# guptakhil/show-tell

Measured on AMD Instinct MI355X. Metric: training images/sec (ResNet101+GRU, emb=512, bs=128) at 1/2/4/8 MI355X, higher is better.
Workload: dtype bf16; 1 GPU; BASELINE configs[1]: ResNet-101 (train-mode BN, frozen) + 5-layer GRU decoder, E=H=512, V=10000, fwd+bwd+SGD step, synthetic COCO-shaped batch; batch_per_gpu=128, global_batch=128, image=3x224x224, parallelism=dp1

## Files before the change

include/showtell_hip.h:

```cpp
#ifndef SHOWTELL_HIP_H
#define SHOWTELL_HIP_H

#include <stddef.h>
#include <stdint.h>

#ifdef __cplusplus
extern "C" {
#endif

#define ST_F32 0
#define ST_BF16 1

#define ST_CELL_GRU 0
#define ST_CELL_LSTM 1

const char* st_last_error(void);
int st_version(void);

typedef struct {
  const void* x;
  const void* w;
  void* y;
  const float* bias;
  const float* scale;
  const float* shift;
  const void* residual;
  float* stats;
  int dtype, out_dtype;
  int B, Hin, Win, Cin, Ho, Wo, N, KH, KW, stride, pad;
  int ldx, ldw, ldy;
  int relu, accumulate;
  int Cin_logical;
  int k_order;
  int stats_replicas;
  const float* in_stats; const float* in_gamma; const float* in_beta; float in_count, in_eps;
  int split_k;
} st_conv_desc;

int st_conv(const st_conv_desc* d, void* stream);
int st_conv_batch(const st_conv_desc* d, int n, void* stream);

typedef struct {
  const void* x; const void* w_frag; void* y;
  float* stats; int stats_replicas;
  const float* scale; const float* shift; int relu;
  const float* in_stats; const float* in_gamma; const float* in_beta; float in_count; float in_eps;
  int B, H, W, C, N;
  int in_stats_replicas;
} st_conv3x3_img_desc;
int st_conv3x3_img_supported(int H, int W, int C, int N);
int st_conv3x3_img(const st_conv3x3_img_desc* d, void* stream);
int st_conv3x3_s2_supported(int C, int N);
int st_conv3x3_s2(const st_conv3x3_img_desc* d, void* stream);
typedef struct {
  const void* x; const void* w_frag; void* y; const void* residual;
  float* stats; int stats_replicas;
  const float* scale; const float* shift; int relu;
  const float* in_stats; const float* in_gamma; const float* in_beta; float in_count; float in_eps; int in_stats_replicas;
  int B, Hin, Win, C, N, stride;
} st_conv1x1_wreg_desc;
int st_conv1x1_wreg_supported(int C, int N);
int st_conv1x1_wreg(const st_conv1x1_wreg_desc* d, void* stream);
int st_conv1x1_kstream_supported(int C, int N);
int st_conv1x1_kstream(const st_conv1x1_wreg_desc* d, void* stream);
typedef struct {
  const void* raw; const void* identity; void* x_out; const void* w_frag; void* y;
  float* stats; int stats_replicas;
  const float* f_stats; const float* f_gamma; const float* f_beta; float f_count; float f_eps; int f_stats_replicas;
  long rows; int C, N;
  const float* id_stats; const float* id_gamma; const float* id_beta; int id_stats_replicas;
} st_conv1x1_kfuse_desc;
int st_conv1x1_kfuse_supported(int C, int N);
int st_conv1x1_kfuse(const st_conv1x1_kfuse_desc* d, void* stream);
#ifdef ST_EXPERIMENTAL
int st_conv1x1_kfuse8(const st_conv1x1_kfuse_desc* d, void* stream);
#endif
typedef struct {
  const void* raw2; const void* w3_frag; const void* identity; void* x_out; const void* w1_frag; void* y;
  float* stats; int stats_replicas;
  const float* bn2_stats; const float* bn2_gamma; const float* bn2_beta; int bn2_replicas;
  const float* bn3_stats; const float* bn3_gamma; const float* bn3_beta; int bn3_replicas;
  const float* id_stats; const float* id_gamma; const float* id_beta; int id_replicas;
  float count; float eps;
  long rows; int C1, C2, N;
} st_conv_b2b_desc;
int st_conv_b2b_supported(int C1, int C2, int N);
int st_conv_b2b(const st_conv_b2b_desc* d, void* stream);
typedef struct {
  const void* x2; const void* w3_frag; const void* identity; void* x_out; const void* w1_frag; void* y;
  float* stats; int stats_replicas;
  const float* bn2_stats; const float* bn2_gamma; const float* bn2_beta; int bn2_replicas;
  const float* bn3_stats; const float* bn3_gamma; const float* bn3_beta; int bn3_replicas;
  float count; float eps;
  const float* scale3; const float* shift3; const float* scale1; const float* shift1; int relu1;
  long rows; int C1, C2, N;
  const float* id_stats; const float* id_gamma; const float* id_beta; int id_replicas;
} st_conv_c3c1_desc;
int st_conv_c3c1_supported(int C1, int C2, int N);
int st_conv_c3c1(const st_conv_c3c1_desc* d, void* stream);
int st_conv1x1_astat_supported(int C, int N);
int st_conv1x1_astat(const st_conv1x1_wreg_desc* d, void* stream);

int st_pack_conv_weight_frag(const float* w, void* out, int Cout, int Cin, int KH, int KW, int ntw, void* stream);

int st_tune(int reserved, int kc, int w8);
int st_prof_enable(int on);
int st_debug_stamps(unsigned long long* buf);
int st_prof_collect(double* ms, double* flops, long* launches);

typedef struct {
  const void* x; void* y; const void* res;
  const float* stats;  const float* gamma; const float* beta;
  const float* running_mean; const float* running_var;
  const float* res_stats; const float* res_gamma; const float* res_beta;
  const float* res_running_mean; const float* res_running_var;
  int res_bn;
  int dtype; long rows; int C; float count; float eps; int relu;
  int stats_replicas, res_stats_replicas;
} st_bn_act_desc;

int st_bn_act(const st_bn_act_desc* d, void* stream);

int st_bn_update_running(const float* stats, float* running_mean, float* running_var,
                         int C, float count, float momentum, void* stream);

int st_nchw_to_nhwc(const float* x, void* y, int dtype, int B, int C, int H, int W, int Cpad, void* stream);
int st_nchw_to_s2d16(const float* x, void* y, int dtype, int B, int H, int W, void* stream);
int st_stem_weight_s2d(const void* w, void* out, int dtype, int Cpad, void* stream);
int st_nhwc_to_ncp_f32(const void* x, float* y, int dtype, int B, int HW, int C, void* stream);
int st_maxpool3x3s2(const void* x, void* y, int dtype, int B, int H, int W, int C, void* stream);
int st_maxpool3x3s2_bn(const void* x, void* y, int dtype, int B, int H, int W, int C,
                       const float* stats, const float* gamma, const float* beta,
                       const float* running_mean, const float* running_var, float count, float eps, void* stream);
typedef struct {
  const void* x_s2d; const void* w_frag; void* y;
  float* stats; int stats_replicas;
  const float* gamma;
  const float* scale; const float* shift;
  int B, H, W;
} st_stem_conv_pool_desc;
int st_stem_conv_pool(const st_stem_conv_pool_desc* d, void* stream);
int st_stem_weight_frag(const void* w_s2d, void* out, void* stream);
int st_stem_weight_frag_packed(const void* w_packed, int Cpad, void* out, void* stream);
int st_global_avgpool(const void* x, void* y, int dtype, int out_dtype, int B, int HW, int C, void* stream);

typedef struct st_image_batch_desc {
  const uint8_t* src;
  int64_t src_bytes;
  const int64_t* offset;
  const int32_t* height;
  const int32_t* width;
  const int32_t* flip;
  int batch;
  int max_height, max_width;
  int out_h, out_w;
  const float* lut;
  uint8_t* tmp;
  float* out;
  uint8_t* out_u8;
} st_image_batch_desc;
int st_image_transform(const st_image_batch_desc* d, void* stream);

int st_cast(const void* x, void* y, int from_dtype, int to_dtype, long n, void* stream);
int st_transpose(const void* x, void* y, int dtype, int rows, int cols, int ldx, int ldy, void* stream);
int st_transpose_colsum(const void* x, void* y, float* colsum, int dtype, int rows, int cols, int ldx, int ldy, void* stream);
int st_transpose_batch(const void* const* x, void* const* y, float* const* colsum, int n, int dtype, int rows, int cols,
                       int ldx, int ldy, const int* rows_t, const int* prev_row, void* stream);
int st_pack_conv_weight(const float* w, void* out, int dtype, int Cout, int Cin, int KH, int KW, int Cpad, int k_order, void* stream);

typedef struct st_resnet st_resnet;
int st_resnet_create(int version, int dtype, st_resnet** out);
void st_resnet_destroy(st_resnet* r);
int st_resnet_num_convs(const st_resnet* r);
int st_resnet_feat_dim(const st_resnet* r);
size_t st_resnet_weight_elems(const st_resnet* r);
size_t st_resnet_bn_channels(const st_resnet* r);
int st_resnet_conv_info(const st_resnet* r, int i, int* cin, int* cout, int* k, int* stride, int* pad,
                        int* cin_padded, size_t* weight_offset, size_t* bn_offset, int* k_order,
                        size_t* frag_weight_offset, int* frag_ntw);
size_t st_resnet_workspace_bytes(const st_resnet* r, int B, int H, int W);
int st_resnet_set_taps(st_resnet* r, void* buf, size_t bytes);
int st_resnet_forward(const st_resnet* r, const float* images_nchw, int B, int H, int W,
                      const void* weights, const float* bn_gamma, const float* bn_beta,
                      float* bn_running_mean, float* bn_running_var,
                      int train, float momentum, float eps,
                      void* workspace, size_t workspace_bytes,
                      void* feat_nhwc_out, void* pooled_out, int pooled_dtype, float* ncp_out,
                      void* stream);

int st_resnet_update_running(const st_resnet* r, const void* workspace, float* bn_running_mean, float* bn_running_var,
                             float momentum, void* stream);
int st_resnet_plan(const st_resnet* r, int B, int H, int W, int train, char* buf, size_t bytes);

int st_cast2d(const void* x, void* y, int from_dtype, int to_dtype, int rows, int cols, int ldx, int ldy, void* stream);

#define ST_MAX_LAYERS 8
typedef struct {
  int cell, dtype, L, in0, H, V, E;
  const void* emb;
  const void* w_ih[ST_MAX_LAYERS]; const void* w_hh[ST_MAX_LAYERS];
  const float* b_ih[ST_MAX_LAYERS]; const float* b_hh[ST_MAX_LAYERS];
  const void* w_lin; const float* b_lin;
} st_rnn_params;

typedef struct {
  float* emb;
  float* w_ih[ST_MAX_LAYERS]; float* w_hh[ST_MAX_LAYERS]; float* b_ih[ST_MAX_LAYERS]; float* b_hh[ST_MAX_LAYERS];
  float* w_lin; float* b_lin;
} st_rnn_grads;

typedef struct {
  int B, T, ntok, Tcap;
  const int* batch_sizes_host;
  const int* rows_b; const int* rows_t; const int* prev_row;
  const long* caption;
} st_packed_seq;

int st_rnn_vocab_ld(int V);
size_t st_rnn_workspace_bytes(const st_rnn_params* p, const st_packed_seq* s);
int st_rnn_forward(const st_rnn_params* p, const st_packed_seq* s, const void* x0_override, const void* feat,
                   void* workspace, size_t workspace_bytes, void* logits, int logits_dtype, int ldl,
                   long* targets, int save_for_backward, void* stream);
int st_rnn_backward(const st_rnn_params* p, const st_rnn_grads* g, const st_packed_seq* s,
                    const void* x0_override, const void* dlogits, int ldd, const float* dy_top,
                    void* workspace, size_t workspace_bytes, float* dfeat, float* dx0_out, void* stream);

int st_rnn_fused_loss_supported(const st_rnn_params* p);
size_t st_rnn_fused_loss_bytes(const st_rnn_params* p, const st_packed_seq* s);
int st_rnn_fused_loss(const st_rnn_params* p, const st_packed_seq* s, const void* workspace, size_t workspace_bytes,
                      const long* targets, float* scratch, size_t scratch_bytes, float* loss_accum, void* stream);
int st_rnn_fused_dlogits(const st_rnn_params* p, const st_packed_seq* s, const void* workspace, size_t workspace_bytes,
                         const long* targets, const float* scratch, const float* grad_scale_dev, void* dlogits, int ldd, void* stream);

int st_cross_entropy(const void* logits, int logits_dtype, const long* target, int rows, int V, int ldl,
                     float* loss_accum, void* dlogits, int dlogits_dtype, int ldd, float grad_scale,
                     const float* grad_scale_dev , void* stream);

size_t st_head_workspace_bytes(int B, int F, int E, int dtype);
int st_linear_bn1d_forward(const void* x, const void* w, const float* bias, const float* gamma, const float* beta,
                           float* running_mean, float* running_var, int B, int F, int E, int dtype,
                           int train, float momentum, float eps,
                           float* z_out, float* save_mean, float* save_rstd, void* y_dtype, float* y_f32, void* stream);
int st_linear_bn1d_backward(const float* dy, const float* z, const void* x, const float* gamma,
                            const float* save_mean, const float* save_rstd, int B, int F, int E, int dtype, int train,
                            float* dw, float* dbias, float* dgamma, float* dbeta, void* workspace, size_t workspace_bytes,
                            void* stream);

int st_sgd_step(float* param, const float* grad, float* momentum_buf, void* bf16_shadow, long n,
                float lr, float momentum, int first_step, float grad_scale, void* stream);
int st_adam_step(float* param, const float* grad, float* exp_avg, float* exp_avg_sq, void* bf16_shadow, long n,
                 float lr, float beta1, float beta2, float eps, int step, float grad_scale, void* stream);

size_t st_rnn_greedy_workspace_bytes(const st_rnn_params* p, int B);
int st_rnn_greedy(const st_rnn_params* p, const void* feat, int B, int steps, void* workspace, size_t workspace_bytes,
                  long* ids_out, float* logits_out, void* stream);
int st_rnn_greedy_last_route(void);

int st_rnn_step(const st_rnn_params* p, const void* x, int n, const void* h_in, const void* c_in,
                void* h_out, void* c_out, float* logits, int ldl, void* stream);
int st_embedding_rows(const void* emb, const long* ids, void* out, int n, int E, int V, int ldo, int dtype, void* stream);
int st_gather_state(const void* src, const int* idx, void* dst, int L, int n_src, int n_dst, int H, int dtype, void* stream);
int st_softmax_topk(const float* logits, int ldl, int n, int V, int k, float* top_p, long* top_id, int raw, void* stream);
int st_beam_select(const long* tok, const float* cost, uint8_t* done, const float* top_p, const long* top_id, int B, int W, int k,
                   long end_id, long* new_tok, float* new_cost, int* parent, uint8_t* ended, int* gather, void* stream);

int st_sample_rows(const float* logits, int ldl, int n, int V, const float* u, int u_stride, float inv_temperature, int top_k,
                   long end_id, uint8_t* finished, long* ids_out, float* logp_out, int out_stride, int t, long* cur, void* stream);
size_t st_rnn_sample_workspace_bytes(const st_rnn_params* p, int n);
int st_rnn_sample(const st_rnn_params* p, const void* feat, int n, int steps, const float* u, float inv_temperature, int top_k,
                  long end_id, void* workspace, size_t workspace_bytes, long* ids_out, float* logp_out, void* stream);

typedef struct {
  st_rnn_params rnn;
  int F, A, P;
  const void* w_enc; const float* b_enc;
  const void* w_dec; const float* b_dec;
  const float* w_full; const float* b_full;
  const void* w_init_h; const float* b_init_h;
  const void* w_init_c; const float* b_init_c;
  const void* w_embed; const float* b_embed;
} st_attn_params;

typedef struct {
  st_rnn_grads rnn;
  float *w_enc, *b_enc, *w_dec, *b_dec, *w_full, *b_full, *w_init_h, *b_init_h, *w_init_c, *b_init_c, *w_embed, *b_embed;
} st_attn_grads;

size_t st_attn_workspace_bytes(const st_attn_params* p, const st_packed_seq* s);
int st_attn_forward(const st_attn_params* p, const st_packed_seq* s, const float* cnn_feature, const long* caption_T,
                    void* workspace, size_t workspace_bytes, void* logits, int logits_dtype, int ldl,
                    float* alphas, int save_for_backward, void* stream);
int st_attn_backward(const st_attn_params* p, const st_attn_grads* g, const st_packed_seq* s, const long* caption_T,
                     const void* dlogits, int ldd, const float* alphas,
                     const float* dalphas ,
                     float alpha_c, const float* grad_scale_dev, void* workspace, size_t workspace_bytes, void* stream);
int st_attn_reg_loss(const float* alphas, int B, int T, int P, float alpha_c, float* loss_accum, void* stream);
size_t st_attn_greedy_workspace_bytes(const st_attn_params* p, int B);
int st_attn_greedy(const st_attn_params* p, const float* cnn_feature, int B, int steps, long start_id,
                   void* workspace, size_t workspace_bytes, long* ids_out, void* stream);
int st_attn_greedy_alphas(const st_attn_params* p, const float* cnn_feature, int B, int steps, long start_id,
                          void* workspace, size_t workspace_bytes, long* ids_out, float* alphas_out, void* stream);
size_t st_attn_sample_workspace_bytes(const st_attn_params* p, int n);
int st_attn_sample(const st_attn_params* p, const float* cnn_feature, int n, int steps, long start_id, const float* u,
                   float inv_temperature, int top_k, long end_id, void* workspace, size_t workspace_bytes,
                   long* ids_out, float* logp_out, float* alphas_out, void* stream);
size_t st_attn_beam_workspace_bytes(const st_attn_params* p, int B, int W);
int st_attn_beam_search(const st_attn_params* p, const float* cnn_feature, int B, int W, int max_length,
                        long start_id, long end_id, void* workspace, size_t workspace_bytes,
                        long* rec_tok, float* rec_cost, int* rec_par, uint8_t* rec_end, float* rec_alpha, void* stream);

#ifdef __cplusplus
}
#endif
#endif
```

show-tell_amd/_lib.py:

```python
import ctypes as C
import os

_HERE = os.path.dirname(os.path.abspath(__file__))
LIB_PATH = os.path.join(_HERE, "lib", "libshowtell_hip.so")

ST_F32, ST_BF16 = 0, 1
ST_CELL_GRU, ST_CELL_LSTM = 0, 1

c_p, c_i, c_f, c_l = C.c_void_p, C.c_int, C.c_float, C.c_long


class ConvDesc(C.Structure):
    _fields_ = [("x", c_p), ("w", c_p), ("y", c_p), ("bias", c_p), ("scale", c_p), ("shift", c_p),
                ("residual", c_p), ("stats", c_p), ("dtype", c_i), ("out_dtype", c_i),
                ("B", c_i), ("Hin", c_i), ("Win", c_i), ("Cin", c_i), ("Ho", c_i), ("Wo", c_i), ("N", c_i),
                ("KH", c_i), ("KW", c_i), ("stride", c_i), ("pad", c_i),
                ("ldx", c_i), ("ldw", c_i), ("ldy", c_i), ("relu", c_i), ("accumulate", c_i), ("Cin_logical", c_i), ("k_order", c_i), ("stats_replicas", c_i),
                ("in_stats", c_p), ("in_gamma", c_p), ("in_beta", c_p), ("in_count", c_f), ("in_eps", c_f), ("split_k", c_i)]


class Conv3x3ImgDesc(C.Structure):
    _fields_ = [("x", c_p), ("w_frag", c_p), ("y", c_p), ("stats", c_p), ("stats_replicas", c_i), ("scale", c_p), ("shift", c_p),
                ("relu", c_i), ("in_stats", c_p), ("in_gamma", c_p), ("in_beta", c_p), ("in_count", c_f), ("in_eps", c_f),
                ("B", c_i), ("H", c_i), ("W", c_i), ("C", c_i), ("N", c_i), ("in_stats_replicas", c_i)]


class Conv1x1WregDesc(C.Structure):
    _fields_ = [("x", c_p), ("w_frag", c_p), ("y", c_p), ("residual", c_p), ("stats", c_p), ("stats_replicas", c_i), ("scale", c_p),
                ("shift", c_p), ("relu", c_i), ("in_stats", c_p), ("in_gamma", c_p), ("in_beta", c_p), ("in_count", c_f), ("in_eps", c_f),
                ("in_stats_replicas", c_i), ("B", c_i), ("Hin", c_i), ("Win", c_i), ("C", c_i), ("N", c_i), ("stride", c_i)]


class Conv1x1KfuseDesc(C.Structure):
    _fields_ = [("raw", c_p), ("identity", c_p), ("x_out", c_p), ("w_frag", c_p), ("y", c_p), ("stats", c_p), ("stats_replicas", c_i),
                ("f_stats", c_p), ("f_gamma", c_p), ("f_beta", c_p), ("f_count", c_f), ("f_eps", c_f), ("f_stats_replicas", c_i),
                ("rows", c_l), ("C", c_i), ("N", c_i),
                ("id_stats", c_p), ("id_gamma", c_p), ("id_beta", c_p), ("id_stats_replicas", c_i)]


class StemConvPoolDesc(C.Structure):
    _fields_ = [("x_s2d", c_p), ("w_frag", c_p), ("y", c_p), ("stats", c_p), ("stats_replicas", c_i), ("gamma", c_p),
                ("scale", c_p), ("shift", c_p), ("B", c_i), ("H", c_i), ("W", c_i)]


class ConvB2bDesc(C.Structure):
    _fields_ = [("raw2", c_p), ("w3_frag", c_p), ("identity", c_p), ("x_out", c_p), ("w1_frag", c_p), ("y", c_p),
                ("stats", c_p), ("stats_replicas", c_i),
                ("bn2_stats", c_p), ("bn2_gamma", c_p), ("bn2_beta", c_p), ("bn2_replicas", c_i),
                ("bn3_stats", c_p), ("bn3_gamma", c_p), ("bn3_beta", c_p), ("bn3_replicas", c_i),
                ("id_stats", c_p), ("id_gamma", c_p), ("id_beta", c_p), ("id_replicas", c_i),
                ("count", c_f), ("eps", c_f), ("rows", c_l), ("C1", c_i), ("C2", c_i), ("N", c_i)]


class ConvC3c1Desc(C.Structure):
    _fields_ = [("x2", c_p), ("w3_frag", c_p), ("identity", c_p), ("x_out", c_p), ("w1_frag", c_p), ("y", c_p),
                ("stats", c_p), ("stats_replicas", c_i),
                ("bn2_stats", c_p), ("bn2_gamma", c_p), ("bn2_beta", c_p), ("bn2_replicas", c_i),
                ("bn3_stats", c_p), ("bn3_gamma", c_p), ("bn3_beta", c_p), ("bn3_replicas", c_i),
                ("count", c_f), ("eps", c_f),
                ("scale3", c_p), ("shift3", c_p), ("scale1", c_p), ("shift1", c_p), ("relu1", c_i),
                ("rows", c_l), ("C1", c_i), ("C2", c_i), ("N", c_i),
                ("id_stats", c_p), ("id_gamma", c_p), ("id_beta", c_p), ("id_replicas", c_i)]


class BnActDesc(C.Structure):
    _fields_ = [("x", c_p), ("y", c_p), ("res", c_p), ("stats", c_p), ("gamma", c_p), ("beta", c_p),
                ("running_mean", c_p), ("running_var", c_p), ("res_stats", c_p), ("res_gamma", c_p),
                ("res_beta", c_p), ("res_running_mean", c_p), ("res_running_var", c_p), ("res_bn", c_i),
                ("dtype", c_i), ("rows", c_l), ("C", c_i), ("count", c_f), ("eps", c_f), ("relu", c_i),
                ("stats_replicas", c_i), ("res_stats_replicas", c_i)]


ST_MAX_LAYERS = 8


class RnnParams(C.Structure):
    _fields_ = [("cell", c_i), ("dtype", c_i), ("L", c_i), ("in0", c_i), ("H", c_i), ("V", c_i), ("E", c_i),
                ("emb", c_p), ("w_ih", c_p * ST_MAX_LAYERS), ("w_hh", c_p * ST_MAX_LAYERS),
                ("b_ih", c_p * ST_MAX_LAYERS), ("b_hh", c_p * ST_MAX_LAYERS), ("w_lin", c_p), ("b_lin", c_p)]


class RnnGrads(C.Structure):
    _fields_ = [("emb", c_p), ("w_ih", c_p * ST_MAX_LAYERS), ("w_hh", c_p * ST_MAX_LAYERS),
                ("b_ih", c_p * ST_MAX_LAYERS), ("b_hh", c_p * ST_MAX_LAYERS), ("w_lin", c_p), ("b_lin", c_p)]


class AttnParams(C.Structure):
    _fields_ = [("rnn", RnnParams), ("F", c_i), ("A", c_i), ("P", c_i),
                ("w_enc", c_p), ("b_enc", c_p), ("w_dec", c_p), ("b_dec", c_p), ("w_full", c_p), ("b_full", c_p),
                ("w_init_h", c_p), ("b_init_h", c_p), ("w_init_c", c_p), ("b_init_c", c_p), ("w_embed", c_p), ("b_embed", c_p)]


class AttnGrads(C.Structure):
    _fields_ = [("rnn", RnnGrads)] + [(n, c_p) for n in ("w_enc", "b_enc", "w_dec", "b_dec", "w_full", "b_full", "w_init_h", "b_init_h",
                                                        "w_init_c", "b_init_c", "w_embed", "b_embed")]


class PackedSeq(C.Structure):
    _fields_ = [("B", c_i), ("T", c_i), ("ntok", c_i), ("Tcap", c_i), ("batch_sizes_host", C.POINTER(c_i)),
                ("rows_b", c_p), ("rows_t", c_p), ("prev_row", c_p), ("caption", c_p)]


class ImageBatchDesc(C.Structure):
    _fields_ = [("src", c_p), ("src_bytes", C.c_int64), ("offset", c_p), ("height", c_p), ("width", c_p), ("flip", c_p), ("batch", c_i),
                ("max_height", c_i), ("max_width", c_i), ("out_h", c_i), ("out_w", c_i), ("lut", c_p), ("tmp", c_p),
                ("out", c_p), ("out_u8", c_p)]


_SIGS = {
    "st_version": ([], c_i),
    "st_image_transform": ([C.POINTER(ImageBatchDesc), c_p], c_i),
    "st_conv": ([C.POINTER(ConvDesc), c_p], c_i),
    "st_conv_batch": ([C.POINTER(ConvDesc), c_i, c_p], c_i),
    "st_conv3x3_img_supported": ([c_i, c_i, c_i, c_i], c_i),
    "st_conv3x3_img": ([C.POINTER(Conv3x3ImgDesc), c_p], c_i),
    "st_conv3x3_s2_supported": ([c_i, c_i], c_i),
    "st_conv3x3_s2": ([C.POINTER(Conv3x3ImgDesc), c_p], c_i),
    "st_conv1x1_wreg_supported": ([c_i, c_i], c_i),
    "st_conv1x1_wreg": ([C.POINTER(Conv1x1WregDesc), c_p], c_i),
    "st_conv1x1_kfuse": ([C.POINTER(Conv1x1KfuseDesc), c_p], c_i),
    "st_conv1x1_kfuse_supported": ([c_i, c_i], c_i),
    "st_conv1x1_kfuse8": ([C.POINTER(Conv1x1KfuseDesc), c_p], c_i),
    "st_conv_b2b": ([C.POINTER(ConvB2bDesc), c_p], c_i),
    "st_conv_b2b_supported": ([c_i, c_i, c_i], c_i),
    "st_conv1x1_astat_supported": ([c_i, c_i], c_i),
    "st_conv1x1_astat": ([C.POINTER(Conv1x1WregDesc), c_p], c_i),
    "st_conv1x1_kstream_supported": ([c_i, c_i], c_i),
    "st_conv1x1_kstream": ([C.POINTER(Conv1x1WregDesc), c_p], c_i),
    "st_pack_conv_weight_frag": ([c_p, c_p, c_i, c_i, c_i, c_i, c_i, c_p], c_i),
    "st_tune": ([c_i, c_i, c_i], c_i),
    "st_prof_enable": ([c_i], c_i),
    "st_debug_stamps": ([c_p], c_i),
    "st_prof_collect": ([C.POINTER(C.c_double), C.POINTER(C.c_double), C.POINTER(c_l)], c_i),
    "st_bn_act": ([C.POINTER(BnActDesc), c_p], c_i),
    "st_bn_update_running": ([c_p, c_p, c_p, c_i, c_f, c_f, c_p], c_i),
    "st_nchw_to_nhwc": ([c_p, c_p, c_i, c_i, c_i, c_i, c_i, c_i, c_p], c_i),
    "st_nchw_to_s2d16": ([c_p, c_p, c_i, c_i, c_i, c_i, c_p], c_i),
    "st_stem_weight_s2d": ([c_p, c_p, c_i, c_i, c_p], c_i),
    "st_stem_weight_frag": ([c_p, c_p, c_p], c_i),
    "st_stem_weight_frag_packed": ([c_p, c_i, c_p, c_p], c_i),
    "st_stem_conv_pool": ([C.POINTER(StemConvPoolDesc), c_p], c_i),
    "st_nhwc_to_ncp_f32": ([c_p, c_p, c_i, c_i, c_i, c_i, c_p], c_i),
    "st_maxpool3x3s2": ([c_p, c_p, c_i, c_i, c_i, c_i, c_i, c_p], c_i),
    "st_maxpool3x3s2_bn": ([c_p, c_p, c_i, c_i, c_i, c_i, c_i, c_p, c_p, c_p, c_p, c_p, c_f, c_f, c_p], c_i),
    "st_global_avgpool": ([c_p, c_p, c_i, c_i, c_i, c_i, c_i, c_p], c_i),
    "st_cast": ([c_p, c_p, c_i, c_i, c_l, c_p], c_i),
    "st_transpose": ([c_p, c_p, c_i, c_i, c_i, c_i, c_i, c_p], c_i),
    "st_transpose_colsum": ([c_p, c_p, c_p, c_i, c_i, c_i, c_i, c_i, c_p], c_i),
    "st_transpose_batch": ([c_p, c_p, c_p, c_i, c_i, c_i, c_i, c_i, c_i, c_p, c_p, c_p], c_i),
    "st_pack_conv_weight": ([c_p, c_p, c_i, c_i, c_i, c_i, c_i, c_i, c_i, c_p], c_i),
    "st_cast2d": ([c_p, c_p, c_i, c_i, c_i, c_i, c_i, c_i, c_p], c_i),
    "st_rnn_vocab_ld": ([c_i], c_i),
    "st_rnn_workspace_bytes": ([C.POINTER(RnnParams), C.POINTER(PackedSeq)], C.c_size_t),
    "st_rnn_forward": ([C.POINTER(RnnParams), C.POINTER(PackedSeq), c_p, c_p, c_p, C.c_size_t, c_p, c_i, c_i, c_p, c_i, c_p], c_i),
    "st_rnn_fused_loss_supported": ([C.POINTER(RnnParams)], c_i),
    "st_rnn_fused_loss_bytes": ([C.POINTER(RnnParams), C.POINTER(PackedSeq)], C.c_size_t),
    "st_rnn_fused_loss": ([C.POINTER(RnnParams), C.POINTER(PackedSeq), c_p, C.c_size_t, c_p, c_p, C.c_size_t, c_p, c_p], c_i),
    "st_rnn_fused_dlogits": ([C.POINTER(RnnParams), C.POINTER(PackedSeq), c_p, C.c_size_t, c_p, c_p, c_p, c_p, c_i, c_p], c_i),
    "st_rnn_backward": ([C.POINTER(RnnParams), C.POINTER(RnnGrads), C.POINTER(PackedSeq), c_p, c_p, c_i, c_p, c_p, C.c_size_t,
                         c_p, c_p, c_p], c_i),
    "st_rnn_greedy_workspace_bytes": ([C.POINTER(RnnParams), c_i], C.c_size_t),
    "st_rnn_greedy": ([C.POINTER(RnnParams), c_p, c_i, c_i, c_p, C.c_size_t, c_p, c_p, c_p], c_i),
    "st_rnn_greedy_last_route": ([], c_i),
    "st_rnn_step": ([C.POINTER(RnnParams), c_p, c_i, c_p, c_p, c_p, c_p, c_p, c_i, c_p], c_i),
    "st_embedding_rows": ([c_p, c_p, c_p, c_i, c_i, c_i, c_i, c_i, c_p], c_i),
    "st_gather_state": ([c_p, c_p, c_p, c_i, c_i, c_i, c_i, c_i, c_p], c_i),
    "st_softmax_topk": ([c_p, c_i, c_i, c_i, c_i, c_p, c_p, c_i, c_p], c_i),
    "st_beam_select": ([c_p, c_p, c_p, c_p, c_p, c_i, c_i, c_i, c_l, c_p, c_p, c_p, c_p, c_p, c_p], c_i),
    "st_sample_rows": ([c_p, c_i, c_i, c_i, c_p, c_i, c_f, c_i, c_l, c_p, c_p, c_p, c_i, c_i, c_p, c_p], c_i),
    "st_rnn_sample_workspace_bytes": ([C.POINTER(RnnParams), c_i], C.c_size_t),
    "st_rnn_sample": ([C.POINTER(RnnParams), c_p, c_i, c_i, c_p, c_f, c_i, c_l, c_p, C.c_size_t, c_p, c_p, c_p], c_i),
    "st_attn_workspace_bytes": ([c_p, c_p], C.c_size_t),
    "st_attn_forward": ([c_p, c_p, c_p, c_p, c_p, C.c_size_t, c_p, c_i, c_i, c_p, c_i, c_p], c_i),
    "st_attn_backward": ([c_p, c_p, c_p, c_p, c_p, c_i, c_p, c_p, c_f, c_p, c_p, C.c_size_t, c_p], c_i),
    "st_attn_reg_loss": ([c_p, c_i, c_i, c_i, c_f, c_p, c_p], c_i),
    "st_attn_greedy_workspace_bytes": ([c_p, c_i], C.c_size_t),
    "st_attn_greedy": ([c_p, c_p, c_i, c_i, c_l, c_p, C.c_size_t, c_p, c_p], c_i),
    "st_attn_greedy_alphas": ([c_p, c_p, c_i, c_i, c_l, c_p, C.c_size_t, c_p, c_p, c_p], c_i),
    "st_attn_sample_workspace_bytes": ([c_p, c_i], C.c_size_t),
    "st_attn_sample": ([c_p, c_p, c_i, c_i, c_l, c_p, c_f, c_i, c_l, c_p, C.c_size_t, c_p, c_p, c_p, c_p], c_i),
    "st_attn_beam_workspace_bytes": ([c_p, c_i, c_i], C.c_size_t),
    "st_attn_beam_search": ([c_p, c_p, c_i, c_i, c_i, c_l, c_l, c_p, C.c_size_t, c_p, c_p, c_p, c_p, c_p, c_p], c_i),
    "st_cross_entropy": ([c_p, c_i, c_p, c_i, c_i, c_i, c_p, c_p, c_i, c_i, c_f, c_p, c_p], c_i),
    "st_head_workspace_bytes": ([c_i, c_i, c_i, c_i], C.c_size_t),
    "st_linear_bn1d_forward": ([c_p] * 7 + [c_i, c_i, c_i, c_i, c_i, c_f, c_f] + [c_p] * 6, c_i),
    "st_linear_bn1d_backward": ([c_p] * 6 + [c_i, c_i, c_i, c_i, c_i] + [c_p] * 5 + [C.c_size_t, c_p], c_i),
    "st_sgd_step": ([c_p, c_p, c_p, c_p, c_l, c_f, c_f, c_i, c_f, c_p], c_i),
    "st_adam_step": ([c_p, c_p, c_p, c_p, c_p, c_l, c_f, c_f, c_f, c_f, c_i, c_f, c_p], c_i),
    "st_resnet_create": ([c_i, c_i, C.POINTER(c_p)], c_i),
    "st_resnet_destroy": ([c_p], None),
    "st_resnet_num_convs": ([c_p], c_i),
    "st_resnet_feat_dim": ([c_p], c_i),
    "st_resnet_weight_elems": ([c_p], C.c_size_t),
    "st_resnet_bn_channels": ([c_p], C.c_size_t),
    "st_resnet_conv_info": ([c_p, c_i] + [C.POINTER(c_i)] * 6 + [C.POINTER(C.c_size_t)] * 2 + [C.POINTER(c_i), C.POINTER(C.c_size_t), C.POINTER(c_i)], c_i),
    "st_resnet_workspace_bytes": ([c_p, c_i, c_i, c_i], C.c_size_t),
    "st_resnet_set_taps": ([c_p, c_p, C.c_size_t], c_i),
    "st_resnet_forward": ([c_p, c_p, c_i, c_i, c_i, c_p, c_p, c_p, c_p, c_p, c_i, c_f, c_f, c_p, C.c_size_t,
                           c_p, c_p, c_i, c_p, c_p], c_i),
    "st_resnet_update_running": ([c_p, c_p, c_p, c_p, c_f, c_p], c_i),
    "st_resnet_plan": ([c_p, c_i, c_i, c_i, c_i, C.c_char_p, C.c_size_t], c_i),
}

_lib = None


class ShowTellHipError(RuntimeError):
    pass


def declared_symbols():
    return sorted([k for k in _SIGS if k not in _EXPERIMENTAL] + ["st_last_error"])


_EXPERIMENTAL = ("st_conv1x1_kfuse8",)


def has_symbol(name):
    return hasattr(lib(), name)


def lib():
    global _lib
    if _lib is None:
        if not os.path.isfile(LIB_PATH):
            raise ShowTellHipError(
                f"{LIB_PATH} not found: build it with `python -c 'import __graft_entry__ as g; g.build()'` "
                "(there is no CPU fallback for the HIP path)")
        import torch
        L = C.CDLL(LIB_PATH)
        L.st_last_error.restype = C.c_char_p
        L.st_last_error.argtypes = []
        for name, (args, res) in _SIGS.items():
            if name in _EXPERIMENTAL and not hasattr(L, name):
                continue
            fn = getattr(L, name)
            fn.argtypes, fn.restype = args, res
        _lib = L
    return _lib


def check(rc, what):
    if rc != 0:
        raise ShowTellHipError(f"{what}: {lib().st_last_error().decode()}")
```

show-tell_amd/csrc/rnn.cpp:

```cpp
#include "decoder_host.h"
#include <stdlib.h>

namespace {

struct Plan {
  int G, GH, Np, Vp, maxw;
  size_t es;
  size_t x0, y, gates, cst, dyl, dx0, dgx, dgh, dhc, dcc, tA, tB, wT, wThh, wTih, gA, gB, total;
};

Plan make_plan(const st_rnn_params* p, const st_packed_seq* s) {
  Plan q;
  q.G = p->cell == ST_CELL_GRU ? 3 : 4;
  q.GH = q.G * p->H;
  q.Np = st_up8(s->ntok);
  q.Vp = st_rnn_vocab_ld(p->V);
  q.es = st_dtype_size(p->dtype);
  q.maxw = p->in0 > p->H ? p->in0 : p->H;
  const size_t n = s->ntok, L = p->L, H = p->H;
  Arena ar;
  q.x0 = ar.take(n * p->in0 * q.es);
  q.y = ar.take(L * n * H * q.es);
  q.gates = ar.take(L * n * 4 * H * q.es);
  q.cst = ar.take(p->cell == ST_CELL_LSTM ? L * n * H * q.es : 0);
  q.dyl = ar.take(L * n * H * sizeof(float));
  q.dx0 = ar.take(n * p->in0 * sizeof(float));
  q.dgx = ar.take(L * n * q.GH * q.es);
  q.dgh = ar.take(p->cell == ST_CELL_GRU ? L * n * q.GH * q.es : 0);
  q.dhc = ar.take(L * (size_t)s->B * H * sizeof(float));
  q.dcc = ar.take(L * (size_t)s->B * H * sizeof(float));
  const size_t ra = (size_t)(p->V > q.GH ? p->V : q.GH);
  q.tA = ar.take(ra * q.Np * q.es);
  q.tB = ar.take((size_t)q.maxw * q.Np * q.es);
  const size_t w1 = (size_t)H * q.Vp, w2 = (size_t)q.maxw * q.GH;
  q.wT = ar.take((w1 > w2 ? w1 : w2) * q.es);
  q.wThh = ar.take(L * H * q.GH * q.es);
  q.wTih = ar.take(L * (size_t)q.maxw * q.GH * q.es);
  q.gA = ar.take(2 * L * (size_t)q.GH * q.Np * q.es);
  q.gB = ar.take(2 * L * (size_t)q.maxw * q.Np * q.es);
  q.total = ar.o;
  return q;
}

int check_common(const st_rnn_params* p, const st_packed_seq* s, const char* who) {
  ST_CHECK(p && s, "%s: null descriptor", who);
  ST_CHECK(p->cell == ST_CELL_GRU || p->cell == ST_CELL_LSTM, "%s: bad cell %d", who, p->cell);
  ST_CHECK(p->dtype == ST_F32 || p->dtype == ST_BF16, "%s: bad dtype %d", who, p->dtype);
  ST_CHECK(p->L >= 1 && p->L <= ST_MAX_LAYERS, "%s: num_layers=%d out of range [1,%d]", who, p->L, ST_MAX_LAYERS);
  ST_CHECK(p->H % 8 == 0 && p->in0 % 8 == 0 && p->E % 8 == 0, "%s: E=%d, in0=%d and H=%d must be multiples of 8", who, p->E, p->in0, p->H);
  ST_CHECK(p->V > 0, "%s: bad vocabulary size", who);
  if (st_check_packed_seq(s, who, true)) return 1;
  for (int l = 0; l < p->L; ++l)
    ST_CHECK(p->w_ih[l] && p->w_hh[l] && p->b_ih[l] && p->b_hh[l], "%s: null weights for layer %d", who, l);
  return 0;
}

}

extern "C" int st_rnn_vocab_ld(int V) { return V < 2048 ? st_up8(V) : (V + 511) / 512 * 512; }

extern "C" size_t st_rnn_workspace_bytes(const st_rnn_params* p, const st_packed_seq* s) {
  if (!p || !s) return 0;
  return make_plan(p, s).total;
}

extern "C" int st_rnn_forward(const st_rnn_params* p, const st_packed_seq* s, const void* x0_override, const void* feat,
                              void* workspace, size_t workspace_bytes, void* logits, int logits_dtype, int ldl,
                              long* targets, int save_for_backward, void* stream) {
  if (check_common(p, s, "st_rnn_forward")) return 1;
  ST_CHECK(workspace && (x0_override || (feat && p->emb)), "st_rnn_forward: null pointer");
  const Plan q = make_plan(p, s);
  ST_CHECK(workspace_bytes >= q.total, "st_rnn_forward: workspace too small (%zu < %zu)", workspace_bytes, q.total);
  hipStream_t st = reinterpret_cast<hipStream_t>(stream);
  char* ws = reinterpret_cast<char*>(workspace);
  const int dt = p->dtype, H = p->H, n = s->ntok;
  const size_t es = q.es;

  const void* x0 = x0_override;
  if (!x0) {
    ST_CHECK(p->in0 == p->E, "st_rnn_forward: in0 != E needs x0_override");
    if (pack_inputs_launch(feat, p->emb, s->caption, s->Tcap, s->rows_b, s->rows_t, ws + q.x0, targets, n, p->E, p->V, 0, dt, st)) return 1;
    x0 = ws + q.x0;
  }
  const std::vector<int> off = st_packed_offsets(s);

  const int L = p->L, T = s->T;
  for (int d = 0; d < T + L - 1; ++d) {
    RnnGemmArgs cells[ST_MAX_LAYERS];
    int nc = 0;
    for (int l = d < T ? 0 : d - (T - 1); l <= d && l < L; ++l) {
      const int t = d - l;
      const int bt = s->batch_sizes_host[t];
      const char* xl = l == 0 ? reinterpret_cast<const char*>(x0) : ws + q.y + (size_t)(l - 1) * n * H * es;
      const int in = l == 0 ? p->in0 : H;
      char* yl = ws + q.y + (size_t)l * n * H * es;
      char* gl = ws + q.gates + (size_t)l * n * 4 * H * es;
      char* cl = ws + q.cst + (size_t)l * n * H * es;
      cells[nc++] = rnn_full_cell(p, l, xl + (size_t)off[t] * in * es, in, t > 0 ? yl + (size_t)off[t - 1] * H * es : nullptr,
                                  t > 0 ? cl + (size_t)off[t - 1] * H * es : nullptr, yl + (size_t)off[t] * H * es, cl + (size_t)off[t] * H * es,
                                  bt, save_for_backward ? gl + (size_t)off[t] * 4 * H * es : nullptr);
    }
    if (rnn_gemm_launch_batch(cells, nc, dt, rnn_cell_epi(p->cell), 1, st)) return 1;
  }
  if (logits) {
    ST_CHECK(p->w_lin && p->b_lin, "st_rnn_forward: logits requested without the vocabulary projection");
    const char* ytop = ws + q.y + (size_t)(p->L - 1) * n * H * es;
    if (st_gemm_nt(ytop, H, p->w_lin, H, logits, ldl, n, p->V, H, dt, logits_dtype, p->b_lin, stream)) return 1;
  }
  return 0;
}

extern "C" int st_rnn_fused_loss_supported(const st_rnn_params* p) {
  return p && p->w_lin && p->b_lin && vocab_ce_supported(p->dtype, p->H) ? 1 : 0;
}
extern "C" size_t st_rnn_fused_loss_bytes(const st_rnn_params* p, const st_packed_seq* s) {
  if (!p || !s) return 0;
  return ((size_t)s->ntok * (2 + 2 * (size_t)vocab_ce_tiles(p->V))) * sizeof(float);
}
extern "C" int st_rnn_fused_loss(const st_rnn_params* p, const st_packed_seq* s, const void* workspace, size_t workspace_bytes,
                                 const long* targets, float* scratch, size_t scratch_bytes, float* loss_accum, void* stream) {
  if (check_common(p, s, "st_rnn_fused_loss")) return 1;
  ST_CHECK(workspace && targets && scratch && loss_accum, "st_rnn_fused_loss: null pointer");
  ST_CHECK(st_rnn_fused_loss_supported(p), "st_rnn_fused_loss: needs bf16, H = 512 and the vocabulary projection (use st_rnn_forward's logits + st_cross_entropy)");
  const Plan q = make_plan(p, s);
  ST_CHECK(workspace_bytes >= q.total && scratch_bytes >= st_rnn_fused_loss_bytes(p, s), "st_rnn_fused_loss: workspace / scratch too small");
  const char* ytop = reinterpret_cast<const char*>(workspace) + q.y + (size_t)(p->L - 1) * s->ntok * p->H * q.es;
  const int n = s->ntok;
  return vocab_ce_forward(ytop, p->w_lin, p->b_lin, targets, n, p->V, scratch + 2 * (size_t)n, scratch + n, scratch, loss_accum,
                          reinterpret_cast<hipStream_t>(stream));
}
extern "C" int st_rnn_fused_dlogits(const st_rnn_params* p, const st_packed_seq* s, const void* workspace, size_t workspace_bytes,
                                    const long* targets, const float* scratch, const float* grad_scale_dev, void* dlogits, int ldd, void* stream) {
  if (check_common(p, s, "st_rnn_fused_dlogits")) return 1;
  ST_CHECK(workspace && targets && scratch && dlogits, "st_rnn_fused_dlogits: null pointer");
  ST_CHECK(st_rnn_fused_loss_supported(p), "st_rnn_fused_dlogits: unsupported configuration");
  const Plan q = make_plan(p, s);
  ST_CHECK(workspace_bytes >= q.total, "st_rnn_fused_dlogits: workspace too small");
  const char* ytop = reinterpret_cast<const char*>(workspace) + q.y + (size_t)(p->L - 1) * s->ntok * p->H * q.es;
  return vocab_ce_dlogits(ytop, p->w_lin, p->b_lin, targets, scratch, s->ntok, p->V, dlogits, ldd, 1.0f, grad_scale_dev,
                          reinterpret_cast<hipStream_t>(stream));
}

extern "C" int st_rnn_backward(const st_rnn_params* p, const st_rnn_grads* g, const st_packed_seq* s,
                               const void* x0_override, const void* dlogits, int ldd, const float* dy_top_extra,
                               void* workspace, size_t workspace_bytes, float* dfeat, float* dx0_out, void* stream) {
  if (check_common(p, s, "st_rnn_backward")) return 1;
  ST_CHECK(g && workspace, "st_rnn_backward: null pointer");
  const Plan q = make_plan(p, s);
  ST_CHECK(workspace_bytes >= q.total, "st_rnn_backward: workspace too small (%zu < %zu)", workspace_bytes, q.total);
  hipStream_t st = reinterpret_cast<hipStream_t>(stream);
  char* ws = reinterpret_cast<char*>(workspace);
  const int dt = p->dtype, H = p->H, n = s->ntok, Np = q.Np, GH = q.GH;
  const size_t es = q.es;
  const std::vector<int> off = st_packed_offsets(s);
  const int L = p->L, T = s->T;
  auto dyl = [&](int l) { return reinterpret_cast<float*>(ws + q.dyl) + (size_t)l * n * H; };
  float* dy = dyl(L - 1);
  const char* ytop = ws + q.y + (size_t)(p->L - 1) * n * H * es;

  if (dlogits) {
    ST_CHECK(p->w_lin && g->w_lin && g->b_lin, "st_rnn_backward: vocabulary projection gradients requested without buffers");
    ST_CHECK(ldd >= st_up8(p->V) && ldd % 8 == 0 && ldd <= q.Vp, "st_rnn_backward: dlogits leading dimension %d must be a multiple of 8 in [%d, %d]",
             ldd, st_up8(p->V), q.Vp);
    if (st_transpose_colsum(dlogits, ws + q.tA, g->b_lin, dt, n, p->V, ldd, Np, stream)) return 1;
    if (st_transpose(ytop, ws + q.tB, dt, n, H, H, Np, stream)) return 1;
    if (st_gemm_nt(ws + q.tA, Np, ws + q.tB, Np, g->w_lin, H, p->V, H, Np, dt, ST_F32, nullptr, stream, 1)) return 1;
    if (st_transpose(p->w_lin, ws + q.wT, dt, p->V, H, H, ldd, stream)) return 1;
    const int bk = dt == ST_BF16 ? 64 : 32;
    const int split = (ldd % (8 * bk) == 0 && ldd >= 16 * bk) ? 8 : 0;
    if (st_gemm_nt(dlogits, ldd, ws + q.wT, ldd, dy, H, n, H, ldd, dt, ST_F32, nullptr, stream, 0, split)) return 1;
    if (dy_top_extra) { st_set_error("st_rnn_backward: dlogits and dy_top_extra are exclusive"); return 1; }
  } else {
    ST_CHECK(dy_top_extra, "st_rnn_backward: need dlogits or dy_top");
    if (hipMemcpyAsync(dy, dy_top_extra, (size_t)n * H * sizeof(float), hipMemcpyDeviceToDevice, st) != hipSuccess) {
      st_set_error("st_rnn_backward: copy failed"); return 1;
    }
  }

  const void* x0 = x0_override ? x0_override : ws + q.x0;
  const bool need_dx0 = dfeat || dx0_out || g->emb;
  float* dx0 = dx0_out ? dx0_out : reinterpret_cast<float*>(ws + q.dx0);
  const bool gru = p->cell == ST_CELL_GRU;
  auto dgxl = [&](int l) { return ws + q.dgx + (size_t)l * n * GH * es; };
  auto dghl = [&](int l) { return gru ? ws + q.dgh + (size_t)l * n * GH * es : dgxl(l); };
  auto dhcl = [&](int l) { return reinterpret_cast<float*>(ws + q.dhc) + (size_t)l * s->B * H; };
  auto dccl = [&](int l) { return reinterpret_cast<float*>(ws + q.dcc) + (size_t)l * s->B * H; };
  auto wThh = [&](int l) { return ws + q.wThh + (size_t)l * H * GH * es; };
  auto wTih = [&](int l) { return ws + q.wTih + (size_t)l * q.maxw * GH * es; };
  if (hipMemsetAsync(ws + q.dhc, 0, (size_t)L * s->B * H * sizeof(float), st) != hipSuccess ||
      hipMemsetAsync(ws + q.dcc, 0, (size_t)L * s->B * H * sizeof(float), st) != hipSuccess) { st_set_error("memset failed"); return 1; }
  {
    const void* wx[2][ST_MAX_LAYERS]; void* wy[2][ST_MAX_LAYERS];
    int ni = 0;
    for (int l = 0; l < L; ++l) {
      const int in = l == 0 ? p->in0 : H;
      wx[0][l] = p->w_hh[l]; wy[0][l] = wThh(l);
      if (!(l > 0 || need_dx0)) continue;
      if (in == H) { wx[1][ni] = p->w_ih[l]; wy[1][ni] = wTih(l); ++ni; }
      else if (st_transpose(p->w_ih[l], wTih(l), dt, GH, in, in, GH, stream)) return 1;
    }
    if (st_transpose_batch(wx[0], wy[0], nullptr, L, dt, GH, H, H, GH, nullptr, nullptr, stream)) return 1;
    if (ni && st_transpose_batch(wx[1], wy[1], nullptr, ni, dt, GH, H, H, GH, nullptr, nullptr, stream)) return 1;
  }
  auto bwd_cell = [&](int l, int t, const float* dyrows) {
    const char* yl = ws + q.y + (size_t)l * n * H * es;
    const char* gl = ws + q.gates + (size_t)l * n * 4 * H * es;
    const char* cl = ws + q.cst + (size_t)l * n * H * es;
    RnnBwdCell c;
    memset(&c, 0, sizeof(c));
    c.dy = dyrows ? dyrows + (size_t)off[t] * H : nullptr; c.dhc = dhcl(l); c.dcc = dccl(l);
    c.cache = gl + (size_t)off[t] * 4 * H * es;
    c.hprev = t > 0 ? yl + (size_t)off[t - 1] * H * es : nullptr;
    c.cnew = cl + (size_t)off[t] * H * es;
    c.cprev = t > 0 ? cl + (size_t)off[t - 1] * H * es : nullptr;
    c.dgx = dgxl(l) + (size_t)off[t] * GH * es; c.dgh = dghl(l) + (size_t)off[t] * GH * es; c.Bt = s->batch_sizes_host[t];
    return c;
  };
  const char* env = getenv("ST_BPTT_FUSED");
  const bool fused = !(env && env[0] == '0');
  for (int d = T + L - 2; fused && d >= 0; --d) {
    RnnBwdFused fc[ST_MAX_LAYERS];
    int nf = 0;
    for (int l = d < T ? 0 : d - (T - 1); l <= d && l < L; ++l) {
      const int t = d - l;
      RnnBwdFused& f = fc[nf++];
      memset(&f, 0, sizeof(f));
      f.e = bwd_cell(l, t, l == L - 1 ? dy : nullptr);
      RnnGemmArgs& a = f.g;
      a.M = f.e.Bt; a.N = H;
      if (t + 1 < T) {
        a.A = dghl(l) + (size_t)off[t + 1] * GH * es; a.W = wThh(l); a.M2 = s->batch_sizes_host[t + 1]; a.K = GH; a.lda = GH; a.ldw = GH;
      }
      if (l + 1 < L) {
        a.A2 = dgxl(l + 1) + (size_t)off[t] * GH * es; a.W2 = wTih(l + 1); a.K2 = GH; a.lda2 = GH; a.ldw2 = GH;
      }
    }
    if (rnn_bwd_fused_launch_batch(fc, nf, p->cell, dt, st)) return 1;
  }
  if (fused && need_dx0 && st_gemm_nt(dgxl(0), GH, wTih(0), GH, dx0, p->in0, n, p->in0, GH, dt, ST_F32, nullptr, stream)) return 1;
  for (int d = T + L - 2; !fused && d >= 0; --d) {
    RnnBwdCell gc[ST_MAX_LAYERS];
    RnnGemmArgs mc[2 * ST_MAX_LAYERS];
    int ng = 0, nm = 0;
    for (int l = d < T ? 0 : d - (T - 1); l <= d && l < L; ++l) {
      const int t = d - l;
      const int bt = s->batch_sizes_host[t];
      const int in = l == 0 ? p->in0 : H;
      gc[ng++] = bwd_cell(l, t, dyl(l));
      if (t > 0) {
        RnnGemmArgs& a = mc[nm++];
        memset(&a, 0, sizeof(a));
        a.A = dghl(l) + (size_t)off[t] * GH * es; a.W = wThh(l); a.M = bt; a.N = H; a.K = GH; a.lda = GH; a.ldw = GH;
        a.out_f32 = dhcl(l); a.ldo = H; a.accumulate = 1;
      }
      if (l > 0 || need_dx0) {
        RnnGemmArgs& a = mc[nm++];
        memset(&a, 0, sizeof(a));
        a.A = dgxl(l) + (size_t)off[t] * GH * es; a.W = wTih(l); a.M = bt; a.N = in; a.K = GH; a.lda = GH; a.ldw = GH;
        a.out_f32 = (l > 0 ? dyl(l - 1) + (size_t)off[t] * H : dx0 + (size_t)off[t] * in); a.ldo = in;
      }
    }
    if (rnn_bwd_gates_launch_batch(gc, ng, H, p->cell, dt, st)) return 1;
    if (rnn_gemm_launch_batch(mc, nm, dt, 0, 0, st)) return 1;
  }
  st_conv_desc gd[2 * ST_MAX_LAYERS];
  int ng = 0;
  auto wgrad = [&](const void* aT, const void* bT, float* dw, int rows, int cols) {
    gd[ng++] = st_gemm_nt_desc(aT, Np, bT, Np, dw, cols, rows, cols, Np, dt, ST_F32, nullptr, 1);
  };
  const void* tx[4][ST_MAX_LAYERS]; void* ty[4][ST_MAX_LAYERS]; float* tc[4][ST_MAX_LAYERS];
  int nx = 0;
  for (int l = 0; l < L; ++l) {
    const int in = l == 0 ? p->in0 : H;
    const char* xl = l == 0 ? reinterpret_cast<const char*>(x0) : ws + q.y + (size_t)(l - 1) * n * H * es;
    char* aIh = ws + q.gA + (size_t)(2 * l) * GH * Np * es;
    char* aHh = ws + q.gA + (size_t)(2 * l + 1) * GH * Np * es;
    char* bIh = ws + q.gB + (size_t)(2 * l) * q.maxw * Np * es;
    char* bHh = ws + q.gB + (size_t)(2 * l + 1) * q.maxw * Np * es;
    tx[0][l] = dgxl(l); ty[0][l] = aIh; tc[0][l] = g->b_ih[l];
    tx[2][l] = dghl(l); ty[2][l] = aHh; tc[2][l] = g->b_hh[l];
    tx[3][l] = ws + q.y + (size_t)l * n * H * es; ty[3][l] = bHh; tc[3][l] = nullptr;
    if (in == H) {
      tx[1][nx] = xl; ty[1][nx] = bIh; tc[1][nx] = nullptr; ++nx;
      wgrad(aIh, bIh, g->w_ih[l], GH, in);
    } else {
      if (st_transpose(xl, bIh, dt, n, in, in, Np, stream)) return 1;
    }
    wgrad(gru ? aHh : aIh, bHh, g->w_hh[l], GH, H);
    if (!gru && colsum_launch(dghl(l), g->b_hh[l], n, GH, GH, dt, st)) return 1;
  }
  if (st_transpose_batch(tx[0], ty[0], tc[0], L, dt, n, GH, GH, Np, nullptr, nullptr, stream)) return 1;
  if (nx && st_transpose_batch(tx[1], ty[1], nullptr, nx, dt, n, H, H, Np, nullptr, nullptr, stream)) return 1;
  if (gru && st_transpose_batch(tx[2], ty[2], tc[2], L, dt, n, GH, GH, Np, nullptr, nullptr, stream)) return 1;
  if (st_transpose_batch(tx[3], ty[3], nullptr, L, dt, n, H, H, Np, s->rows_t, s->prev_row, stream)) return 1;
  for (int l = 0; l < L; ++l) {
    const int in = l == 0 ? p->in0 : H;
    if (in != H && st_gemm_nt(ws + q.gA + (size_t)(2 * l) * GH * Np * es, Np, ws + q.gB + (size_t)(2 * l) * q.maxw * Np * es, Np,
                              g->w_ih[l], in, GH, in, Np, dt, ST_F32, nullptr, stream, 1)) return 1;
  }
  for (int i = 0; i < ng; i += 12) {
    if (st_conv_batch(gd + i, ng - i < 12 ? ng - i : 12, stream)) return 1;
  }
  if (need_dx0 && !x0_override) {
    ST_CHECK(g->emb, "st_rnn_backward: embedding gradient buffer missing");
    if (embedding_bwd_launch(dx0, s->caption, s->Tcap, s->rows_b, s->rows_t, dfeat, g->emb, n, p->E, p->V, 0, st)) return 1;
  }
  return 0;
}
```

show-tell_amd/csrc/rnn_kernels.h:

```cpp
#pragma once
#include "common.h"

struct RnnGemmArgs {
  const void* A; const void* W; int M, N, K, lda, ldw, gstride;
  const void* A2; const void* W2; int K2, lda2, ldw2;
  int M2;
  float* out_f32; int ldo; int accumulate;
  const float* bias_h; const float* bias_x;
  const void* gx; int ldgx;
  const void* hprev; const void* cprev; int ldhp;
  void* hout; void* cout; int ldho;
  void* hout2; int ldho2;
  void* cache; int ldcache;
  unsigned long long* argmax_keys;
  const unsigned long long* x_keys; int x_V;
  long* ids_out; int ids_stride, ids_t;
};
constexpr int kCellRawOut = 1, kCellSplit = 2;

constexpr int kRnnBatch = 16;
struct RnnGemmBatch { RnnGemmArgs c[kRnnBatch]; };
static_assert(sizeof(RnnGemmBatch) <= 4000, "kernel-argument segment is 4 KiB");
struct RnnBwdCell {
  const float* dy; float* dhc; float* dcc; const void* cache; const void* hprev; const void* cnew; const void* cprev;
  void* dgx; void* dgh; int Bt;
};
struct RnnBwdBatch { RnnBwdCell c[kRnnBatch]; };
struct RnnBwdFused { RnnGemmArgs g; RnnBwdCell e; };
struct RnnBwdFusedBatch { RnnBwdFused c[ST_MAX_LAYERS]; };
static_assert(sizeof(RnnBwdFusedBatch) <= 4000, "kernel-argument segment is 4 KiB");

#ifdef __HIPCC__
__device__ __forceinline__ float st_sigm(float x) { return 1.0f / (1.0f + expf(-x)); }
__device__ __forceinline__ float st_gru_unit(float xr, float xz, float xn, float hr, float hz, float hn, float hprev, float& r, float& z, float& n) {
  r = st_sigm(xr + hr);
  z = st_sigm(xz + hz);
  n = tanhf(__builtin_fmaf(r, hn, xn));
  return __builtin_fmaf(z, hprev, (1.f - z) * n);
}
__device__ __forceinline__ float st_lstm_unit(float pi, float pf, float pg, float po, float cprev, float& ig, float& fg, float& gg, float& og, float& cn) {
  ig = st_sigm(pi); fg = st_sigm(pf); gg = tanhf(pg); og = st_sigm(po);
  cn = __builtin_fmaf(fg, cprev, ig * gg);
  return og * tanhf(cn);
}
#endif

size_t rnn_greedy_pipe_bytes(const st_rnn_params* p, int B, int steps);
int rnn_greedy_pipe(const st_rnn_params* p, const void* feat, int B, int steps, void* ws, size_t ws_bytes, long* ids_out, hipStream_t st);

int vocab_ce_supported(int dtype, int H);
int vocab_ce_tiles(int V);
int vocab_ce_forward(const void* y, const void* w, const float* bias, const long* target, int n, int V, float* partial, float* tgt,
                     float* lse, float* loss, hipStream_t st);
int vocab_ce_dlogits(const void* y, const void* w, const float* bias, const long* target, const float* lse, int n, int V,
                     void* dlogits, int ldd, float gscale, const float* gscale_dev, hipStream_t st);

int rnn_gemm_launch(const RnnGemmArgs& a, int dtype, int epi, int has_x, hipStream_t st);
int rnn_gemm_launch_batch(const RnnGemmArgs* cells, int ncells, int dtype, int epi, int has_x, hipStream_t st);
int rnn_bwd_gates_launch_batch(const RnnBwdCell* cells, int ncells, int H, int cell_kind, int dtype, hipStream_t st);
int rnn_bwd_fused_launch_batch(const RnnBwdFused* cells, int ncells, int cell_kind, int dtype, hipStream_t st);
int pack_inputs_launch(const void* feat, const void* emb, const long* cap, int Tcap, const int* rows_b, const int* rows_t,
                       void* x0, long* target, int ntok, int E, int V, int mode, int dtype, hipStream_t st);
int embedding_bwd_launch(const float* dx0, const long* cap, int Tcap, const int* rows_b, const int* rows_t,
                         float* dfeat, float* demb, int ntok, int E, int V, int mode, hipStream_t st);
int gather_hprev_launch(const void* y, const int* rows_t, const int* prev_row, void* hp, int ntok, int H, int dtype, hipStream_t st,
                        const void* h0 = nullptr, const int* rows_b = nullptr);
int gru_bwd_gates_launch(const float* dy, float* dhc, const void* cache, const void* hprev, void* dgx, void* dgh,
                         int Bt, int H, int dtype, hipStream_t st);
int lstm_bwd_gates_launch(const float* dy, float* dhc, float* dcc, const void* cache, const void* cnew, const void* cprev,
                          void* dg, int Bt, int H, int dtype, hipStream_t st);
int colsum_launch(const void* x, float* out, int rows, int cols, int ldx, int dtype, hipStream_t st);
```

show-tell_amd/csrc/rnn_kernels.hip:

```cpp
#include "common.h"
#include "rnn_kernels.h"
#include <string.h>

namespace {

template <typename T> struct Mfma;
template <> struct Mfma<bf16_t> {
  static constexpr int EPC = 8;
  static __device__ __forceinline__ void run(const u32x4& a, const u32x4& b, f32x4& c) {
    c = __builtin_amdgcn_mfma_f32_16x16x32_bf16(*reinterpret_cast<const bf16x8*>(&a),
                                                *reinterpret_cast<const bf16x8*>(&b), c, 0, 0, 0);
  }
};
template <> struct Mfma<float> {
  static constexpr int EPC = 4;
  static __device__ __forceinline__ void run(const u32x4& a, const u32x4& b, f32x4& c) {
#pragma unroll
    for (int e = 0; e < 4; ++e)
      c = __builtin_amdgcn_mfma_f32_16x16x4f32(__uint_as_float(a[e]), __uint_as_float(b[e]), c, 0, 0, 0);
  }
};

template <typename T> __device__ __forceinline__ void load4(const T* p, float* v);
template <> __device__ __forceinline__ void load4<float>(const float* p, float* v) {
  const f32x4 t = *reinterpret_cast<const f32x4*>(p);
  v[0] = t[0]; v[1] = t[1]; v[2] = t[2]; v[3] = t[3];
}
template <> __device__ __forceinline__ void load4<bf16_t>(const bf16_t* p, float* v) {
  const u32x2 t = *reinterpret_cast<const u32x2*>(p);
  v[0] = __uint_as_float(t[0] << 16); v[1] = __uint_as_float(t[0] & 0xffff0000u);
  v[2] = __uint_as_float(t[1] << 16); v[3] = __uint_as_float(t[1] & 0xffff0000u);
}
template <typename T> __device__ __forceinline__ void store4(T* p, const float* v);
template <> __device__ __forceinline__ void store4<float>(float* p, const float* v) {
  *reinterpret_cast<f32x4*>(p) = f32x4{v[0], v[1], v[2], v[3]};
}
template <> __device__ __forceinline__ void store4<bf16_t>(bf16_t* p, const float* v) {
  *reinterpret_cast<u32x2*>(p) = u32x2{pack_bf16x2(v[0], v[1]), pack_bf16x2(v[2], v[3])};
}

__device__ __forceinline__ float sigm(float x) { return 1.0f / (1.0f + expf(-x)); }

__device__ __forceinline__ u32x4 lane_gather(const u32x4& v, int src4) {
  return u32x4{(unsigned)__builtin_amdgcn_ds_bpermute(src4, (int)v[0]), (unsigned)__builtin_amdgcn_ds_bpermute(src4, (int)v[1]),
               (unsigned)__builtin_amdgcn_ds_bpermute(src4, (int)v[2]), (unsigned)__builtin_amdgcn_ds_bpermute(src4, (int)v[3])};
}
template <typename T, int NG, bool HAS_X, int MT, bool BWD = false>
__device__ __forceinline__ void skinny_mma(const RnnGemmArgs& a, int mbase, int n0, int r16, int q4, int kslice,
                                           f32x4 (&accH)[MT][NG], f32x4 (&accX)[MT][NG]) {
  constexpr int EPC = Mfma<T>::EPC;
  constexpr int UNR = BWD ? (MT + NG <= 4 ? 4 : 2) : (HAS_X && MT == 2) ? 2 : 4;
  const int lr = BWD ? q4 * 4 + (r16 >> 2) : r16, lq = BWD ? (r16 & 3) : q4;
  const int n = n0 + lr;
  const bool nok = n < a.N;
  const bool hasH = a.A != nullptr, hasX = HAS_X && a.A2 != nullptr;
  const T* WH = reinterpret_cast<const T*>(a.W) + (long)n * a.ldw;
  const long gsH = (long)a.gstride * a.ldw;
  const T* WX = reinterpret_cast<const T*>(a.W2) + (long)n * a.ldw2;
  const long gsX = (long)a.gstride * a.ldw2;
  const T* AH[MT]; const T* AX[MT]; bool mok[MT], mokH[MT];
#pragma unroll
  for (int t = 0; t < MT; ++t) {
    const int m = mbase + t * 16 + lr;
    mok[t] = m < a.M;
    mokH[t] = BWD ? m < a.M2 : mok[t];
    AH[t] = reinterpret_cast<const T*>(a.A) + (long)m * a.lda;
    if (!HAS_X && a.x_keys && a.A) {
      int tok = 0;
      if (mok[t]) {
        tok = (int)(0xffffffffu - (unsigned)(a.x_keys[m] & 0xffffffffull));
        if (tok < 0 || tok >= a.x_V) tok = 0;
        if (a.ids_out && n0 == 0 && kslice == 0 && q4 == 0) a.ids_out[(long)m * a.ids_stride + a.ids_t] = tok;
      }
      AH[t] = reinterpret_cast<const T*>(a.A) + (long)tok * a.lda;
    }
    long xrow = m;
    if (HAS_X && a.x_keys) {
      int tok = 0;
      if (mok[t]) {
        tok = (int)(0xffffffffu - (unsigned)(a.x_keys[m] & 0xffffffffull));
        if (tok < 0 || tok >= a.x_V) tok = 0;
        if (a.ids_out && n0 == 0 && kslice == 0 && q4 == 0) a.ids_out[(long)m * a.ids_stride + a.ids_t] = tok;
      }
      xrow = tok;
    }
    AX[t] = reinterpret_cast<const T*>(a.A2) + xrow * a.lda2;
  }
  const int nsH = hasH ? (a.K + 4 * EPC - 1) / (4 * EPC) : 0, nsX = hasX ? (a.K2 + 4 * EPC - 1) / (4 * EPC) : 0;
  const int spwH = (nsH + 3) / 4, spwX = (nsX + 3) / 4;
  const int begH = kslice * spwH, endH = min(nsH, begH + spwH), begX = kslice * spwX, endX = min(nsX, begX + spwX);
  const int ngroups = max((endH - begH + UNR - 1) / UNR, (endX - begX + UNR - 1) / UNR);
  for (int gi = 0; gi < ngroups; ++gi) {
    u32x4 fa[MT][UNR], fw[UNR][NG], xa[MT][UNR], xw[UNR][NG];
#pragma unroll
    for (int u = 0; u < UNR; ++u) {
      const int sH = begH + gi * UNR + u, kH = (sH * 4 + lq) * EPC;
      const bool okH = sH < endH && kH < a.K;
#pragma unroll
      for (int t = 0; t < MT; ++t) {
        fa[t][u] = u32x4{0u, 0u, 0u, 0u};
        if (mokH[t] && okH) fa[t][u] = *reinterpret_cast<const u32x4*>(AH[t] + kH);
      }
#pragma unroll
      for (int g = 0; g < NG; ++g) {
        fw[u][g] = u32x4{0u, 0u, 0u, 0u};
        if ((BWD ? n + g * 16 < a.N : nok) && okH) fw[u][g] = *reinterpret_cast<const u32x4*>(WH + g * gsH + kH);
      }
      if (HAS_X) {
        const int sX = begX + gi * UNR + u, kX = (sX * 4 + lq) * EPC;
        const bool okX = sX < endX && kX < a.K2;
#pragma unroll
        for (int t = 0; t < MT; ++t) {
          xa[t][u] = u32x4{0u, 0u, 0u, 0u};
          if (mok[t] && okX) xa[t][u] = *reinterpret_cast<const u32x4*>(AX[t] + kX);
        }
#pragma unroll
        for (int g = 0; g < NG; ++g) {
          xw[u][g] = u32x4{0u, 0u, 0u, 0u};
          if ((BWD ? n + g * 16 < a.N : nok) && okX) xw[u][g] = *reinterpret_cast<const u32x4*>(WX + g * gsX + kX);
        }
      }
    }
    if (BWD) {
      const int src4 = (r16 * 4 + q4) * 4;
#pragma unroll
      for (int u = 0; u < UNR; ++u) {
#pragma unroll
        for (int t = 0; t < MT; ++t) { fa[t][u] = lane_gather(fa[t][u], src4); xa[t][u] = lane_gather(xa[t][u], src4); }
#pragma unroll
        for (int g = 0; g < NG; ++g) { fw[u][g] = lane_gather(fw[u][g], src4); xw[u][g] = lane_gather(xw[u][g], src4); }
      }
    }
#pragma unroll
    for (int u = 0; u < UNR; ++u)
#pragma unroll
      for (int g = 0; g < NG; ++g)
#pragma unroll
        for (int t = 0; t < MT; ++t) {
          Mfma<T>::run(fw[u][g], fa[t][u], accH[t][g]);
          if (HAS_X) Mfma<T>::run(xw[u][g], xa[t][u], accX[t][g]);
        }
  }
}

template <typename T, int NG, int EPI, bool HAS_X, int MT>
__global__ __launch_bounds__(256) void rnn_gemm_kernel(RnnGemmBatch batch) {
  const RnnGemmArgs& a = batch.c[blockIdx.z];
  __shared__ f32x4 red[4][MT][2 * NG][64];
  const int lane = threadIdx.x & 63;
  const int wid = __builtin_amdgcn_readfirstlane(threadIdx.x >> 6);
  const int r16 = lane & 15, q4 = lane >> 4;
  const int n0 = blockIdx.x * 16, mbase = blockIdx.y * 16 * MT;
  if (mbase >= a.M || n0 >= a.N) return;
  const int m0 = mbase + (wid < MT ? wid : 0) * 16;
  f32x4 accH[MT][NG], accX[MT][NG];
#pragma unroll
  for (int t = 0; t < MT; ++t)
#pragma unroll
    for (int g = 0; g < NG; ++g) { accH[t][g] = f32x4{0.f, 0.f, 0.f, 0.f}; accX[t][g] = f32x4{0.f, 0.f, 0.f, 0.f}; }
  const int pm = m0 + r16, pn = n0 + 4 * q4;
  const bool epi_ok = wid < MT && pm < a.M && pn < a.N && EPI != 3;
  float ex[NG][4], eb[NG][4], es[4] = {0.f, 0.f, 0.f, 0.f};
#pragma unroll
  for (int g = 0; g < NG; ++g)
#pragma unroll
    for (int e = 0; e < 4; ++e) { ex[g][e] = 0.f; eb[g][e] = 0.f; }
  if (epi_ok) {
    if (EPI == 0) {
      if (a.bias_h) load4<float>(a.bias_h + pn, eb[0]);
      if (a.accumulate) load4<float>(a.out_f32 + (long)pm * a.ldo + pn, es);
    } else {
#pragma unroll
      for (int g = 0; g < NG; ++g) {
        load4<float>(a.bias_h + g * a.N + pn, eb[g]);
        if (HAS_X) load4<float>(a.bias_x + g * a.N + pn, ex[g]);
        else if (a.accumulate == kCellSplit) load4<float>(reinterpret_cast<const float*>(a.gx) + (long)pm * a.ldgx + g * a.N + pn, ex[g]);
        else if (a.accumulate != kCellRawOut) load4<T>(reinterpret_cast<const T*>(a.gx) + (long)pm * a.ldgx + g * a.N + pn, ex[g]);
      }
      const void* prev = EPI == 1 ? a.hprev : a.cprev;
      if (prev && a.accumulate != kCellRawOut) load4<T>(reinterpret_cast<const T*>(prev) + (long)pm * a.ldhp + pn, es);
    }
  }
  skinny_mma<T, NG, HAS_X, MT>(a, mbase, n0, r16, q4, wid, accH, accX);
#pragma unroll
  for (int t = 0; t < MT; ++t)
#pragma unroll
    for (int g = 0; g < NG; ++g) { red[wid][t][g][lane] = accH[t][g]; if (HAS_X) red[wid][t][NG + g][lane] = accX[t][g]; }
  __syncthreads();
  if (wid >= MT) return;
  f32x4 sumH[NG], sumX[NG];
#pragma unroll
  for (int g = 0; g < NG; ++g) {
    sumH[g] = red[0][wid][g][lane];
    if (HAS_X) sumX[g] = red[0][wid][NG + g][lane];
#pragma unroll
    for (int w = 1; w < 4; ++w) {
      sumH[g] += red[w][wid][g][lane];
      if (HAS_X) sumX[g] += red[w][wid][NG + g][lane];
    }
  }

  const int m = m0 + r16, n = n0 + 4 * q4;
  if (EPI != 3 && (m >= a.M || n >= a.N)) return;
  const int H = a.N;
  if (EPI == 3) {
    float best = -INFINITY; int bi = 0x7fffffff;
#pragma unroll
    for (int e = 0; e < 4; ++e) {
      if (n + e < a.N) {
        const float v = sumH[0][e] + (a.bias_h ? a.bias_h[n + e] : 0.f);
        if (v > best) { best = v; bi = n + e; }
      }
    }
#pragma unroll
    for (int o = 16; o < 64; o <<= 1) {
      const float ov = __shfl_xor(best, o, 64); const int oi = __shfl_xor(bi, o, 64);
      if (ov > best || (ov == best && oi < bi)) { best = ov; bi = oi; }
    }
    if (q4 == 0 && bi != 0x7fffffff && m < a.M) {
      unsigned u = __float_as_uint(best);
      u = (u & 0x80000000u) ? ~u : (u | 0x80000000u);
      const unsigned long long key = ((unsigned long long)u << 32) | (unsigned long long)(0xffffffffu - (unsigned)bi);
      atomicMax(a.argmax_keys + m, key);
    }
    return;
  }
  if (EPI == 0) {
    float v[4];
#pragma unroll
    for (int e = 0; e < 4; ++e) v[e] = sumH[0][e] + eb[0][e] + es[e];
    if (a.hout) store4<T>(reinterpret_cast<T*>(a.hout) + (long)m * a.ldho + n, v);
    else *reinterpret_cast<f32x4*>(a.out_f32 + (long)m * a.ldo + n) = f32x4{v[0], v[1], v[2], v[3]};
  } else if (!HAS_X && a.accumulate == kCellRawOut) {
#pragma unroll
    for (int g = 0; g < NG; ++g)
      *reinterpret_cast<f32x4*>(a.out_f32 + (long)m * a.ldo + g * a.N + n) =
          f32x4{sumH[g][0] + eb[g][0], sumH[g][1] + eb[g][1], sumH[g][2] + eb[g][2], sumH[g][3] + eb[g][3]};
  } else if (EPI == 1) {
    float xg[3][4];
    const float* hp = es;
    const bool split = !HAS_X && a.accumulate == kCellSplit;
#pragma unroll
    for (int g = 0; g < 3; ++g)
#pragma unroll
      for (int e = 0; e < 4; ++e) xg[g][e] = split ? sumH[g][e] + eb[g][e] : (HAS_X ? sumX[g][e] : 0.f) + ex[g][e];
    float hn[4], r[4], z[4], nn[4], hnew[4];
#pragma unroll
    for (int e = 0; e < 4; ++e) {
      const float hr = split ? ex[0][e] : sumH[0][e] + eb[0][e], hz = split ? ex[1][e] : sumH[1][e] + eb[1][e];
      hn[e] = split ? ex[2][e] : sumH[2][e] + eb[2][e];
      hnew[e] = st_gru_unit(xg[0][e], xg[1][e], xg[2][e], hr, hz, hn[e], hp[e], r[e], z[e], nn[e]);
    }
    store4<T>(reinterpret_cast<T*>(a.hout) + (long)m * a.ldho + n, hnew);
    if (a.hout2) store4<T>(reinterpret_cast<T*>(a.hout2) + (long)m * a.ldho2 + n, hnew);
    if (a.cache) {
      T* c = reinterpret_cast<T*>(a.cache) + (long)m * a.ldcache + n;
      store4<T>(c, r); store4<T>(c + H, z); store4<T>(c + 2 * H, nn); store4<T>(c + 3 * H, hn);
    }
  } else {
    float pre[4][4];
    const float* cp = es;
#pragma unroll
    for (int g = 0; g < 4; ++g)
#pragma unroll
      for (int e = 0; e < 4; ++e) pre[g][e] = (HAS_X ? sumX[g][e] : 0.f) + ex[g < NG ? g : 0][e] + sumH[g < NG ? g : 0][e] + eb[g < NG ? g : 0][e];
    float ig[4], fg[4], gg[4], og[4], cn[4], hnew[4];
#pragma unroll
    for (int e = 0; e < 4; ++e) hnew[e] = st_lstm_unit(pre[0][e], pre[1][e], pre[2][e], pre[3][e], cp[e], ig[e], fg[e], gg[e], og[e], cn[e]);
    store4<T>(reinterpret_cast<T*>(a.hout) + (long)m * a.ldho + n, hnew);
    if (a.hout2) store4<T>(reinterpret_cast<T*>(a.hout2) + (long)m * a.ldho2 + n, hnew);
    store4<T>(reinterpret_cast<T*>(a.cout) + (long)m * a.ldho + n, cn);
    if (a.cache) {
      T* c = reinterpret_cast<T*>(a.cache) + (long)m * a.ldcache + n;
      store4<T>(c, ig); store4<T>(c + H, fg); store4<T>(c + 2 * H, gg); store4<T>(c + 3 * H, og);
    }
  }
}

template <typename T>
__global__ __launch_bounds__(256) void pack_inputs_kernel(const T* __restrict__ feat, const T* __restrict__ emb,
                                                          const long* __restrict__ cap, int Tcap,
                                                          const int* __restrict__ rows_b, const int* __restrict__ rows_t,
                                                          T* __restrict__ x0, long* __restrict__ target,
                                                          int ntok, int E, int V, int mode) {
  constexpr int N = 16 / (int)sizeof(T);
  const int cpr = E / N;
  const long total = (long)ntok * cpr;
  for (long i = (long)blockIdx.x * blockDim.x + threadIdx.x; i < total; i += (long)gridDim.x * blockDim.x) {
    const int row = (int)(i / cpr), c = (int)(i - (long)row * cpr) * N;
    const int b = rows_b[row], t = rows_t[row];
    const T* src;
    if (mode == 0 && t == 0) src = feat + (long)b * E + c;
    else {
      long tok = cap[(long)b * Tcap + (mode == 0 ? t - 1 : t)];
      tok = tok < 0 ? 0 : (tok >= V ? V - 1 : tok);
      src = emb + tok * E + c;
    }
    *reinterpret_cast<u32x4*>(x0 + (long)row * E + c) = *reinterpret_cast<const u32x4*>(src);
    if (c == 0 && target) target[row] = cap[(long)b * Tcap + t];
  }
}

__global__ __launch_bounds__(256) void embedding_bwd_kernel(const float* __restrict__ dx0, const long* __restrict__ cap, int Tcap,
                                                            const int* __restrict__ rows_b, const int* __restrict__ rows_t,
                                                            float* __restrict__ dfeat, float* __restrict__ demb,
                                                            int ntok, int E, int V, int mode) {
  const long total = (long)ntok * E;
  for (long i = (long)blockIdx.x * blockDim.x + threadIdx.x; i < total; i += (long)gridDim.x * blockDim.x) {
    const int row = (int)(i / E), c = (int)(i - (long)row * E);
    const int b = rows_b[row], t = rows_t[row];
    const float v = dx0[i];
    if (mode == 0 && t == 0) { if (dfeat) dfeat[(long)b * E + c] = v; }
    else {
      long tok = cap[(long)b * Tcap + (mode == 0 ? t - 1 : t)];
      tok = tok < 0 ? 0 : (tok >= V ? V - 1 : tok);
      atomicAdd(demb + tok * E + c, v);
    }
  }
}

template <typename T>
__global__ __launch_bounds__(256) void gather_hprev_kernel(const T* __restrict__ y, const int* __restrict__ rows_t,
                                                           const int* __restrict__ prev_row, T* __restrict__ hp, int ntok, int H,
                                                           const T* __restrict__ h0, const int* __restrict__ rows_b) {
  constexpr int N = 16 / (int)sizeof(T);
  const int cpr = H / N;
  const long total = (long)ntok * cpr;
  for (long i = (long)blockIdx.x * blockDim.x + threadIdx.x; i < total; i += (long)gridDim.x * blockDim.x) {
    const int row = (int)(i / cpr), c = (int)(i - (long)row * cpr) * N;
    u32x4 v = {0u, 0u, 0u, 0u};
    if (rows_t[row] > 0) v = *reinterpret_cast<const u32x4*>(y + (long)prev_row[row] * H + c);
    else if (h0) v = *reinterpret_cast<const u32x4*>(h0 + (long)rows_b[row] * H + c);
    *reinterpret_cast<u32x4*>(hp + (long)row * H + c) = v;
  }
}

template <typename T>
__global__ __launch_bounds__(256) void gru_bwd_gates_kernel(RnnBwdBatch batch, int H) {
  const RnnBwdCell& cl = batch.c[blockIdx.y];
  const float* __restrict__ dy = cl.dy; float* __restrict__ dhc = cl.dhc;
  const T* __restrict__ cache = reinterpret_cast<const T*>(cl.cache);
  const T* __restrict__ hprev = reinterpret_cast<const T*>(cl.hprev);
  T* __restrict__ dgx = reinterpret_cast<T*>(cl.dgx); T* __restrict__ dgh = reinterpret_cast<T*>(cl.dgh);
  const int Bt = cl.Bt;
  const int total = Bt * (H / 4);
  const int i = blockIdx.x * blockDim.x + threadIdx.x;
  if (i >= total) return;
  const int b = i / (H / 4), j = (i - b * (H / 4)) * 4;
  float g[4], c[4], r[4], z[4], n[4], hn[4], hp[4] = {0.f, 0.f, 0.f, 0.f};
  load4<float>(dy + (long)b * H + j, g);
  load4<float>(dhc + (long)b * H + j, c);
  const T* cr = cache + (long)b * 4 * H + j;
  load4<T>(cr, r); load4<T>(cr + H, z); load4<T>(cr + 2 * H, n); load4<T>(cr + 3 * H, hn);
  if (hprev) load4<T>(hprev + (long)b * H + j, hp);
  float drp[4], dzp[4], dnp[4], dnr[4], dhz[4];
#pragma unroll
  for (int e = 0; e < 4; ++e) {
    const float dh = g[e] + c[e];
    const float dn = dh * (1.f - z[e]);
    const float dz = dh * (hp[e] - n[e]);
    dnp[e] = dn * (1.f - n[e] * n[e]);
    drp[e] = dnp[e] * hn[e] * r[e] * (1.f - r[e]);
    dzp[e] = dz * z[e] * (1.f - z[e]);
    dnr[e] = dnp[e] * r[e];
    dhz[e] = dh * z[e];
  }
  T* ox = dgx + (long)b * 3 * H + j;
  T* oh = dgh + (long)b * 3 * H + j;
  store4<T>(ox, drp); store4<T>(ox + H, dzp); store4<T>(ox + 2 * H, dnp);
  store4<T>(oh, drp); store4<T>(oh + H, dzp); store4<T>(oh + 2 * H, dnr);
  store4<float>(dhc + (long)b * H + j, dhz);
}

template <typename T>
__global__ __launch_bounds__(256) void lstm_bwd_gates_kernel(RnnBwdBatch batch, int H) {
  const RnnBwdCell& cl = batch.c[blockIdx.y];
  const float* __restrict__ dy = cl.dy; float* __restrict__ dhc = cl.dhc; float* __restrict__ dcc = cl.dcc;
  const T* __restrict__ cache = reinterpret_cast<const T*>(cl.cache);
  const T* __restrict__ cnew = reinterpret_cast<const T*>(cl.cnew);
  const T* __restrict__ cprev = reinterpret_cast<const T*>(cl.cprev);
  T* __restrict__ dg = reinterpret_cast<T*>(cl.dgx);
  const int Bt = cl.Bt;
  const int total = Bt * (H / 4);
  const int i = blockIdx.x * blockDim.x + threadIdx.x;
  if (i >= total) return;
  const int b = i / (H / 4), j = (i - b * (H / 4)) * 4;
  float g[4], ch[4], cc[4], ig[4], fg[4], gg[4], og[4], cn[4], cp[4] = {0.f, 0.f, 0.f, 0.f};
  load4<float>(dy + (long)b * H + j, g);
  load4<float>(dhc + (long)b * H + j, ch);
  load4<float>(dcc + (long)b * H + j, cc);
  const T* cr = cache + (long)b * 4 * H + j;
  load4<T>(cr, ig); load4<T>(cr + H, fg); load4<T>(cr + 2 * H, gg); load4<T>(cr + 3 * H, og);
  load4<T>(cnew + (long)b * H + j, cn);
  if (cprev) load4<T>(cprev + (long)b * H + j, cp);
  float di[4], df[4], dgg[4], dob[4], dcp[4], zero[4] = {0.f, 0.f, 0.f, 0.f};
#pragma unroll
  for (int e = 0; e < 4; ++e) {
    const float dh = g[e] + ch[e];
    const float tc = tanhf(cn[e]);
    const float dc = cc[e] + dh * og[e] * (1.f - tc * tc);
    dob[e] = dh * tc * og[e] * (1.f - og[e]);
    di[e] = dc * gg[e] * ig[e] * (1.f - ig[e]);
    df[e] = dc * cp[e] * fg[e] * (1.f - fg[e]);
    dgg[e] = dc * ig[e] * (1.f - gg[e] * gg[e]);
    dcp[e] = dc * fg[e];
  }
  T* o = dg + (long)b * 4 * H + j;
  store4<T>(o, di); store4<T>(o + H, df); store4<T>(o + 2 * H, dgg); store4<T>(o + 3 * H, dob);
  store4<float>(dcc + (long)b * H + j, dcp);
  store4<float>(dhc + (long)b * H + j, zero);
}


template <typename T> struct Raw4;
template <> struct Raw4<float> { typedef f32x4 type; };
template <> struct Raw4<bf16_t> { typedef u32x2 type; };
template <typename T> __device__ __forceinline__ void unpack4(const typename Raw4<T>::type& t, float* v);
template <> __device__ __forceinline__ void unpack4<float>(const f32x4& t, float* v) { v[0] = t[0]; v[1] = t[1]; v[2] = t[2]; v[3] = t[3]; }
template <> __device__ __forceinline__ void unpack4<bf16_t>(const u32x2& t, float* v) {
  v[0] = __uint_as_float(t[0] << 16); v[1] = __uint_as_float(t[0] & 0xffff0000u);
  v[2] = __uint_as_float(t[1] << 16); v[3] = __uint_as_float(t[1] & 0xffff0000u);
}

template <typename T, bool LSTM, int MT, int NT>
__global__ __launch_bounds__(256) void rnn_bwd_cell_kernel(RnnBwdFusedBatch batch) {
  typedef typename Raw4<T>::type raw_t;
  const RnnGemmArgs& a = batch.c[blockIdx.z].g;
  const RnnBwdCell& c = batch.c[blockIdx.z].e;
  constexpr int TILES = MT * NT, TPW = (TILES + 3) / 4;
  __shared__ f32x4 red[4][TILES][64];
  const int lane = threadIdx.x & 63;
  const int wid = __builtin_amdgcn_readfirstlane(threadIdx.x >> 6);
  const int r16 = lane & 15, q4 = lane >> 4;
  const int n0 = blockIdx.x * 16 * NT, mbase = blockIdx.y * 16 * MT;
  if (mbase >= a.M || n0 >= a.N) return;
  const int H = a.N;
  f32x4 accH[MT][NT], accX[MT][NT];
#pragma unroll
  for (int t = 0; t < MT; ++t)
#pragma unroll
    for (int g = 0; g < NT; ++g) { accH[t][g] = f32x4{0.f, 0.f, 0.f, 0.f}; accX[t][g] = f32x4{0.f, 0.f, 0.f, 0.f}; }
  bool ok[TPW]; int pm[TPW], pn[TPW];
  f32x4 rdy[TPW], rdhc[TPW], rdcc[TPW]; raw_t rc[TPW][4], rp[TPW], rcn[TPW];
  const T* cache = reinterpret_cast<const T*>(c.cache);
#pragma unroll
  for (int j = 0; j < TPW; ++j) {
    const int i = wid + 4 * j;
    pm[j] = mbase + (i / NT) * 16 + r16; pn[j] = n0 + (i % NT) * 16 + 4 * q4;
    ok[j] = i < TILES && pm[j] < a.M && pn[j] < H;
    rdy[j] = rdhc[j] = rdcc[j] = f32x4{0.f, 0.f, 0.f, 0.f};
    rp[j] = rcn[j] = raw_t{};
#pragma unroll
    for (int q = 0; q < 4; ++q) rc[j][q] = raw_t{};
    if (!ok[j]) continue;
    const long o = (long)pm[j] * H + pn[j];
    if (c.dy) rdy[j] = *reinterpret_cast<const f32x4*>(c.dy + o);
#pragma unroll
    for (int q = 0; q < 4; ++q) rc[j][q] = *reinterpret_cast<const raw_t*>(cache + (long)pm[j] * 4 * H + q * H + pn[j]);
    if (LSTM) {
      rdcc[j] = *reinterpret_cast<const f32x4*>(c.dcc + o);
      rcn[j] = *reinterpret_cast<const raw_t*>(reinterpret_cast<const T*>(c.cnew) + o);
      if (c.cprev) rp[j] = *reinterpret_cast<const raw_t*>(reinterpret_cast<const T*>(c.cprev) + o);
    } else {
      rdhc[j] = *reinterpret_cast<const f32x4*>(c.dhc + o);
      if (c.hprev) rp[j] = *reinterpret_cast<const raw_t*>(reinterpret_cast<const T*>(c.hprev) + o);
    }
  }
  skinny_mma<T, NT, true, MT, true>(a, mbase, n0, r16, q4, wid, accH, accX);
#pragma unroll
  for (int t = 0; t < MT; ++t)
#pragma unroll
    for (int g = 0; g < NT; ++g) red[wid][t * NT + g][lane] = accH[t][g] + accX[t][g];
  __syncthreads();
#pragma unroll
  for (int j = 0; j < TPW; ++j) {
    if (!ok[j]) continue;
    const int i = wid + 4 * j;
    const f32x4 s = ((red[0][i][lane] + red[1][i][lane]) + red[2][i][lane]) + red[3][i][lane];
    const long o = (long)pm[j] * H + pn[j];
    if (!LSTM) {
      float r[4], z[4], n[4], hn[4], hp[4];
      unpack4<T>(rc[j][0], r); unpack4<T>(rc[j][1], z); unpack4<T>(rc[j][2], n); unpack4<T>(rc[j][3], hn); unpack4<T>(rp[j], hp);
      float drp[4], dzp[4], dnp[4], dnr[4], dhz[4];
#pragma unroll
      for (int e = 0; e < 4; ++e) {
        const float dh = (rdy[j][e] + rdhc[j][e]) + s[e];
        const float dn = dh * (1.f - z[e]);
        const float dz = dh * (hp[e] - n[e]);
        dnp[e] = dn * (1.f - n[e] * n[e]);
        drp[e] = dnp[e] * hn[e] * r[e] * (1.f - r[e]);
        dzp[e] = dz * z[e] * (1.f - z[e]);
        dnr[e] = dnp[e] * r[e];
        dhz[e] = dh * z[e];
      }
      T* ox = reinterpret_cast<T*>(c.dgx) + (long)pm[j] * 3 * H + pn[j];
      T* oh = reinterpret_cast<T*>(c.dgh) + (long)pm[j] * 3 * H + pn[j];
      store4<T>(ox, drp); store4<T>(ox + H, dzp); store4<T>(ox + 2 * H, dnp);
      store4<T>(oh, drp); store4<T>(oh + H, dzp); store4<T>(oh + 2 * H, dnr);
      store4<float>(c.dhc + o, dhz);
    } else {
      float ig[4], fg[4], gg[4], og[4], cn[4], cp[4];
      unpack4<T>(rc[j][0], ig); unpack4<T>(rc[j][1], fg); unpack4<T>(rc[j][2], gg); unpack4<T>(rc[j][3], og);
      unpack4<T>(rcn[j], cn); unpack4<T>(rp[j], cp);
      float di[4], df[4], dgg[4], dob[4], dcp[4];
#pragma unroll
      for (int e = 0; e < 4; ++e) {
        const float dh = rdy[j][e] + s[e];
        const float tc = tanhf(cn[e]);
        const float dc = rdcc[j][e] + dh * og[e] * (1.f - tc * tc);
        dob[e] = dh * tc * og[e] * (1.f - og[e]);
        di[e] = dc * gg[e] * ig[e] * (1.f - ig[e]);
        df[e] = dc * cp[e] * fg[e] * (1.f - fg[e]);
        dgg[e] = dc * ig[e] * (1.f - gg[e] * gg[e]);
        dcp[e] = dc * fg[e];
      }
      T* og_ = reinterpret_cast<T*>(c.dgx) + (long)pm[j] * 4 * H + pn[j];
      store4<T>(og_, di); store4<T>(og_ + H, df); store4<T>(og_ + 2 * H, dgg); store4<T>(og_ + 3 * H, dob);
      store4<float>(c.dcc + o, dcp);
    }
  }
}

template <typename TL, typename TD>
__global__ __launch_bounds__(256) void ce_kernel(const TL* __restrict__ logits, const long* __restrict__ target,
                                                 float* __restrict__ loss, TD* __restrict__ dlogits,
                                                 int V, int ldl, int ldd, float inv_rows, float gscale, const float* __restrict__ gscale_dev) {
  __shared__ float sm[8], ss[8];
  const int row = blockIdx.x;
  const TL* x = logits + (long)row * ldl;
  float m = -INFINITY, s = 0.f;
  for (int i = threadIdx.x; i < V; i += blockDim.x) {
    const float v = to_f32<TL>(x[i]);
    const float nm = fmaxf(m, v);
    s = s * __expf(m - nm) + __expf(v - nm);
    m = nm;
  }
#pragma unroll
  for (int o = 32; o > 0; o >>= 1) {
    const float om = __shfl_xor(m, o, 64), os = __shfl_xor(s, o, 64);
    const float nm = fmaxf(m, om);
    s = (m == -INFINITY ? 0.f : s * __expf(m - nm)) + (om == -INFINITY ? 0.f : os * __expf(om - nm));
    m = nm;
  }
  const int lane = threadIdx.x & 63, wid = threadIdx.x >> 6;
  if (lane == 0) { sm[wid] = m; ss[wid] = s; }
  __syncthreads();
  float M = sm[0], S = ss[0];
  for (int w = 1; w < (int)(blockDim.x >> 6); ++w) {
    const float nm = fmaxf(M, sm[w]);
    S = S * __expf(M - nm) + ss[w] * __expf(sm[w] - nm);
    M = nm;
  }
  long t = target[row];
  t = t < 0 ? 0 : (t >= V ? V - 1 : t);
  const float lse = M + __logf(S);
  const float xt = to_f32<TL>(x[t]);
  __syncthreads();
  if (threadIdx.x == 0 && loss) atomicAdd(loss, (lse - xt) * inv_rows);
  if (dlogits) {
    if (gscale_dev) gscale *= *gscale_dev;
    TD* d = dlogits + (long)row * ldd;
    for (int i = threadIdx.x; i < V; i += blockDim.x) {
      const float p = __expf(to_f32<TL>(x[i]) - lse);
      d[i] = from_f32<TD>((p - (i == t ? 1.f : 0.f)) * gscale);
    }
    for (int i = V + threadIdx.x; i < ldd; i += blockDim.x) d[i] = from_f32<TD>(0.f);
  }
}

template <typename T>
__global__ __launch_bounds__(256) void colsum_kernel(const T* __restrict__ x, float* __restrict__ out, int rows, int cols, int ldx, int rows_per_block) {
  const int n = blockIdx.x * blockDim.x + threadIdx.x;
  if (n >= cols) return;
  const int r0 = blockIdx.y * rows_per_block, r1 = min(rows, r0 + rows_per_block);
  float s = 0.f;
  for (int r = r0; r < r1; ++r) s += to_f32<T>(x[(long)r * ldx + n]);
  atomicAdd(out + n, s);
}

}

int rnn_gemm_launch_batch(const RnnGemmArgs* cells, int ncells, int dtype, int epi, int has_x, hipStream_t st) {
  ST_CHECK(ncells >= 0 && ncells <= kRnnBatch, "rnn_gemm: %d cells in one launch (max %d)", ncells, kRnnBatch);
  RnnGemmBatch b;
  memset(&b, 0, sizeof(b));
  const int epc = dtype == ST_BF16 ? 8 : 4;
  int nc = 0, maxM = 0, maxN = 0;
  for (int i = 0; i < ncells; ++i) {
    const RnnGemmArgs& a = cells[i];
    if (a.M <= 0) continue;
    ST_CHECK(epi == 3 || a.N % 4 == 0, "rnn_gemm: N=%d must be a multiple of 4", a.N);
    ST_CHECK(a.K % epc == 0 && a.lda % epc == 0 && a.ldw % epc == 0, "rnn_gemm: K/lda/ldw must be multiples of %d", epc);
    if (has_x) ST_CHECK(a.K2 % epc == 0 && a.lda2 % epc == 0 && a.ldw2 % epc == 0, "rnn_gemm: K2/lda2/ldw2 must be multiples of %d", epc);
    b.c[nc++] = a;
    if (a.M > maxM) maxM = a.M;
    if (a.N > maxN) maxN = a.N;
  }
  if (nc == 0) return 0;
  const dim3 grid((maxN + 15) / 16, (maxM + 15) / 16, nc), block(256);
  const bool mt2 = (nc >= 2 || maxM >= 512) && maxM > 16 && epi != 3;
  const dim3 grid2((maxN + 15) / 16, (maxM + 31) / 32, nc);
#define RG(T, NG, EPI, HX) do { if (mt2) hipLaunchKernelGGL((rnn_gemm_kernel<T, NG, EPI, HX, 2>), grid2, block, 0, st, b); \
                               else hipLaunchKernelGGL((rnn_gemm_kernel<T, NG, EPI, HX, 1>), grid, block, 0, st, b); } while (0)
  if (dtype == ST_BF16) {
    if (epi == 0) RG(bf16_t, 1, 0, false);
    else if (epi == 3) RG(bf16_t, 1, 3, false);
    else if (epi == 1) { if (has_x) RG(bf16_t, 3, 1, true); else RG(bf16_t, 3, 1, false); }
    else { if (has_x) RG(bf16_t, 4, 2, true); else RG(bf16_t, 4, 2, false); }
  } else {
    if (epi == 0) RG(float, 1, 0, false);
    else if (epi == 3) RG(float, 1, 3, false);
    else if (epi == 1) { if (has_x) RG(float, 3, 1, true); else RG(float, 3, 1, false); }
    else { if (has_x) RG(float, 4, 2, true); else RG(float, 4, 2, false); }
  }
#undef RG
  ST_LAUNCH_CHECK();
  return 0;
}

int rnn_gemm_launch(const RnnGemmArgs& a, int dtype, int epi, int has_x, hipStream_t st) {
  return rnn_gemm_launch_batch(&a, 1, dtype, epi, has_x, st);
}

int rnn_bwd_gates_launch_batch(const RnnBwdCell* cells, int ncells, int H, int cell_kind, int dtype, hipStream_t st) {
  ST_CHECK(ncells >= 0 && ncells <= kRnnBatch, "rnn_bwd_gates: %d cells in one launch (max %d)", ncells, kRnnBatch);
  RnnBwdBatch b;
  memset(&b, 0, sizeof(b));
  int nc = 0, maxB = 0;
  for (int i = 0; i < ncells; ++i) {
    if (cells[i].Bt <= 0) continue;
    b.c[nc++] = cells[i];
    if (cells[i].Bt > maxB) maxB = cells[i].Bt;
  }
  if (nc == 0) return 0;
  const dim3 grid((maxB * (H / 4) + 255) / 256, nc);
  if (cell_kind == ST_CELL_GRU) {
    if (dtype == ST_BF16) hipLaunchKernelGGL(gru_bwd_gates_kernel<bf16_t>, grid, dim3(256), 0, st, b, H);
    else hipLaunchKernelGGL(gru_bwd_gates_kernel<float>, grid, dim3(256), 0, st, b, H);
  } else {
    if (dtype == ST_BF16) hipLaunchKernelGGL(lstm_bwd_gates_kernel<bf16_t>, grid, dim3(256), 0, st, b, H);
    else hipLaunchKernelGGL(lstm_bwd_gates_kernel<float>, grid, dim3(256), 0, st, b, H);
  }
  ST_LAUNCH_CHECK();
  return 0;
}

int rnn_bwd_fused_launch_batch(const RnnBwdFused* cells, int ncells, int cell_kind, int dtype, hipStream_t st) {
  ST_CHECK(ncells >= 0 && ncells <= ST_MAX_LAYERS, "rnn_bwd_fused: %d cells in one launch (max %d)", ncells, ST_MAX_LAYERS);
  RnnBwdFusedBatch b;
  memset(&b, 0, sizeof(b));
  const int epc = dtype == ST_BF16 ? 8 : 4;
  int nc = 0, maxM = 0, maxN = 0;
  for (int i = 0; i < ncells; ++i) {
    const RnnGemmArgs& a = cells[i].g;
    if (a.M <= 0) continue;
    ST_CHECK(a.N % 8 == 0, "rnn_bwd_fused: H=%d must be a multiple of 8", a.N);
    ST_CHECK(!a.A || (a.K % epc == 0 && a.lda % epc == 0 && a.ldw % epc == 0 && a.M2 >= 0 && a.M2 <= a.M),
             "rnn_bwd_fused: bad recurrent operand pair");
    ST_CHECK(!a.A2 || (a.K2 % epc == 0 && a.lda2 % epc == 0 && a.ldw2 % epc == 0), "rnn_bwd_fused: bad input operand pair");
    b.c[nc] = cells[i];
    b.c[nc].g.gstride = 16;
    if (!a.A) b.c[nc].g.M2 = 0;
    ++nc;
    if (a.M > maxM) maxM = a.M;
    if (a.N > maxN) maxN = a.N;
  }
  if (nc == 0) return 0;
  const bool lstm = cell_kind == ST_CELL_LSTM;
  constexpr int MT = 2, NT = 2;
  const dim3 grid((maxN + 16 * NT - 1) / (16 * NT), (maxM + 16 * MT - 1) / (16 * MT), nc), block(256);
  if (dtype == ST_BF16) {
    if (lstm) hipLaunchKernelGGL((rnn_bwd_cell_kernel<bf16_t, true, MT, NT>), grid, block, 0, st, b);
    else hipLaunchKernelGGL((rnn_bwd_cell_kernel<bf16_t, false, MT, NT>), grid, block, 0, st, b);
  } else {
    if (lstm) hipLaunchKernelGGL((rnn_bwd_cell_kernel<float, true, MT, NT>), grid, block, 0, st, b);
    else hipLaunchKernelGGL((rnn_bwd_cell_kernel<float, false, MT, NT>), grid, block, 0, st, b);
  }
  ST_LAUNCH_CHECK();
  return 0;
}

static inline int grid1d(long work, int threads = 256) {
  long b = (work + threads - 1) / threads;
  return (int)(b < 1 ? 1 : (b > 4096 ? 4096 : b));
}

int pack_inputs_launch(const void* feat, const void* emb, const long* cap, int Tcap, const int* rows_b, const int* rows_t,
                       void* x0, long* target, int ntok, int E, int V, int mode, int dtype, hipStream_t st) {
  if (ntok <= 0) return 0;
  const int n = dtype == ST_BF16 ? 8 : 4;
  ST_CHECK(E % n == 0, "pack_inputs: E=%d must be a multiple of %d", E, n);
  const int grid = grid1d((long)ntok * (E / n));
  if (dtype == ST_BF16) hipLaunchKernelGGL(pack_inputs_kernel<bf16_t>, dim3(grid), dim3(256), 0, st, (const bf16_t*)feat, (const bf16_t*)emb, cap, Tcap, rows_b, rows_t, (bf16_t*)x0, target, ntok, E, V, mode);
  else hipLaunchKernelGGL(pack_inputs_kernel<float>, dim3(grid), dim3(256), 0, st, (const float*)feat, (const float*)emb, cap, Tcap, rows_b, rows_t, (float*)x0, target, ntok, E, V, mode);
  ST_LAUNCH_CHECK();
  return 0;
}

int embedding_bwd_launch(const float* dx0, const long* cap, int Tcap, const int* rows_b, const int* rows_t,
                         float* dfeat, float* demb, int ntok, int E, int V, int mode, hipStream_t st) {
  if (ntok <= 0) return 0;
  hipLaunchKernelGGL(embedding_bwd_kernel, dim3(grid1d((long)ntok * E)), dim3(256), 0, st, dx0, cap, Tcap, rows_b, rows_t, dfeat, demb, ntok, E, V, mode);
  ST_LAUNCH_CHECK();
  return 0;
}

int gather_hprev_launch(const void* y, const int* rows_t, const int* prev_row, void* hp, int ntok, int H, int dtype, hipStream_t st,
                        const void* h0, const int* rows_b) {
  if (ntok <= 0) return 0;
  const int n = dtype == ST_BF16 ? 8 : 4;
  ST_CHECK(H % n == 0, "gather_hprev: H=%d must be a multiple of %d", H, n);
  const int grid = grid1d((long)ntok * (H / n));
  if (dtype == ST_BF16) hipLaunchKernelGGL(gather_hprev_kernel<bf16_t>, dim3(grid), dim3(256), 0, st, (const bf16_t*)y, rows_t, prev_row, (bf16_t*)hp, ntok, H, (const bf16_t*)h0, rows_b);
  else hipLaunchKernelGGL(gather_hprev_kernel<float>, dim3(grid), dim3(256), 0, st, (const float*)y, rows_t, prev_row, (float*)hp, ntok, H, (const float*)h0, rows_b);
  ST_LAUNCH_CHECK();
  return 0;
}

int gru_bwd_gates_launch(const float* dy, float* dhc, const void* cache, const void* hprev, void* dgx, void* dgh,
                         int Bt, int H, int dtype, hipStream_t st) {
  RnnBwdCell c;
  memset(&c, 0, sizeof(c));
  c.dy = dy; c.dhc = dhc; c.cache = cache; c.hprev = hprev; c.dgx = dgx; c.dgh = dgh; c.Bt = Bt;
  return rnn_bwd_gates_launch_batch(&c, 1, H, ST_CELL_GRU, dtype, st);
}

int lstm_bwd_gates_launch(const float* dy, float* dhc, float* dcc, const void* cache, const void* cnew, const void* cprev,
                          void* dg, int Bt, int H, int dtype, hipStream_t st) {
  RnnBwdCell c;
  memset(&c, 0, sizeof(c));
  c.dy = dy; c.dhc = dhc; c.dcc = dcc; c.cache = cache; c.cnew = cnew; c.cprev = cprev; c.dgx = dg; c.Bt = Bt;
  return rnn_bwd_gates_launch_batch(&c, 1, H, ST_CELL_LSTM, dtype, st);
}

int colsum_launch(const void* x, float* out, int rows, int cols, int ldx, int dtype, hipStream_t st) {
  if (rows <= 0 || cols <= 0) return 0;
  const int rpb = 64;
  const dim3 grid((cols + 255) / 256, (rows + rpb - 1) / rpb);
  if (dtype == ST_BF16) hipLaunchKernelGGL(colsum_kernel<bf16_t>, grid, dim3(256), 0, st, (const bf16_t*)x, out, rows, cols, ldx, rpb);
  else hipLaunchKernelGGL(colsum_kernel<float>, grid, dim3(256), 0, st, (const float*)x, out, rows, cols, ldx, rpb);
  ST_LAUNCH_CHECK();
  return 0;
}

extern "C" int st_cross_entropy(const void* logits, int logits_dtype, const long* target, int rows, int V, int ldl,
                                float* loss_accum, void* dlogits, int dlogits_dtype, int ldd, float grad_scale,
                                const float* grad_scale_dev, void* stream) {
  ST_CHECK(logits && target, "st_cross_entropy: null pointer");
  ST_CHECK(rows >= 0 && V > 0 && ldl >= V, "st_cross_entropy: bad shape");
  if (rows == 0) return 0;
  hipStream_t st = reinterpret_cast<hipStream_t>(stream);
  const float inv = 1.0f / rows, gs = grad_scale / rows;
  const dim3 grid(rows), block(256);
  if (logits_dtype == ST_F32 && (dlogits_dtype == ST_F32 || !dlogits))
    hipLaunchKernelGGL((ce_kernel<float, float>), grid, block, 0, st, (const float*)logits, target, loss_accum, (float*)dlogits, V, ldl, ldd, inv, gs, grad_scale_dev);
  else if (logits_dtype == ST_F32)
    hipLaunchKernelGGL((ce_kernel<float, bf16_t>), grid, block, 0, st, (const float*)logits, target, loss_accum, (bf16_t*)dlogits, V, ldl, ldd, inv, gs, grad_scale_dev);
  else if (dlogits_dtype == ST_BF16 || !dlogits)
    hipLaunchKernelGGL((ce_kernel<bf16_t, bf16_t>), grid, block, 0, st, (const bf16_t*)logits, target, loss_accum, (bf16_t*)dlogits, V, ldl, ldd, inv, gs, grad_scale_dev);
  else
    hipLaunchKernelGGL((ce_kernel<bf16_t, float>), grid, block, 0, st, (const bf16_t*)logits, target, loss_accum, (float*)dlogits, V, ldl, ldd, inv, gs, grad_scale_dev);
  ST_LAUNCH_CHECK();
  return 0;
}
```

show-tell_amd/csrc/vocab_ce.hip:

```cpp
#include "common.h"
#include "rnn_kernels.h"

namespace {

constexpr int VH = 512;
constexpr int VPIX = 2 * VH + 32;
constexpr int VTM = 2, VBM = 16 * VTM;
constexpr int VNL = VBM * 64 / 256;
constexpr int VNT = 2;
constexpr int VBN = 64 * VNT;
constexpr int VKS = VH / 32;
constexpr int VSROW = VBN * 2 + 16;
constexpr int VTILE = VBM * VPIX;
constexpr int VLDS = VTILE + 4 * VBM * 2 * 4;

struct VceArgs {
  const bf16_t* y;
  const bf16_t* w;
  const float* bias;
  const long* target;
  float* partial;
  float* tgt_logit;
  const float* lse;
  bf16_t* dlogits;
  const float* gscale_dev; float gscale;
  int n, V, ntile, ldd, nsplit;
};

__device__ __forceinline__ f32x4 vmfma(const u32x4& a, const u32x4& b, const f32x4& c) {
  return __builtin_amdgcn_mfma_f32_16x16x32_bf16(*reinterpret_cast<const bf16x8*>(&a), *reinterpret_cast<const bf16x8*>(&b), c, 0, 0, 0);
}

template <int MODE>
__global__ __launch_bounds__(256, 2) void vocab_ce_kernel(VceArgs a) {
  extern __shared__ __attribute__((aligned(16))) char smem[];
  float* xch = reinterpret_cast<float*>(smem + VTILE);
  char* stage = smem;
  const int tid = threadIdx.x, lane = tid & 63;
  const int wid = __builtin_amdgcn_readfirstlane(tid >> 6);
  const int r16 = lane & 15, q4 = lane >> 4;
  const int mtiles = (a.n + VBM - 1) / VBM;
  const int nt = blockIdx.x / a.nsplit, sp = blockIdx.x - nt * a.nsplit;
  const int n0 = nt * VBN;
  if (sp >= mtiles) return;

  u32x4 tv[VNL];
  auto tile_request = [&](int mt) {
#pragma unroll
    for (int i = 0; i < VNL; ++i) {
      const int c = tid + 256 * i, row = c >> 6, ch = c & 63;
      int m = mt * VBM + row; m = m < a.n ? m : a.n - 1;
      tv[i] = *reinterpret_cast<const u32x4*>(a.y + (size_t)m * VH + ch * 8);
    }
  };
  auto tile_store = [&]() {
#pragma unroll
    for (int i = 0; i < VNL; ++i) { const int c = tid + 256 * i; *reinterpret_cast<u32x4*>(smem + (c >> 6) * VPIX + (c & 63) * 16) = tv[i]; }
  };
  tile_request(sp);
  u32x4 wf[VNT][VKS];
#pragma unroll
  for (int j = 0; j < VNT; ++j) {
    int r = n0 + wid * 32 + 16 * j + r16; r = r < a.V ? r : a.V - 1;
    const bf16_t* wp = a.w + (size_t)r * VH + q4 * 8;
#pragma unroll
    for (int ks = 0; ks < VKS; ++ks) wf[j][ks] = *reinterpret_cast<const u32x4*>(wp + ks * 32);
  }
  float bz[VNT][4]; bool vok[VNT][4];
#pragma unroll
  for (int j = 0; j < VNT; ++j)
#pragma unroll
    for (int e = 0; e < 4; ++e) {
      const int v = n0 + wid * 32 + 16 * j + 4 * q4 + e;
      vok[j][e] = v < a.V;
      bz[j][e] = vok[j][e] ? a.bias[v] : 0.f;
    }
  float gs = a.gscale;
  if (MODE == 1 && a.gscale_dev) gs *= *a.gscale_dev;
  tile_store();
  __syncthreads();

  for (int mt = sp; mt < mtiles; mt += a.nsplit) {
    const int m0 = mt * VBM;
    const bool more = mt + a.nsplit < mtiles;
    if (more) tile_request(mt + a.nsplit);
    f32x4 acc[VTM][VNT];
#pragma unroll
    for (int i = 0; i < VTM; ++i)
#pragma unroll
      for (int j = 0; j < VNT; ++j) acc[i][j] = f32x4{0.f, 0.f, 0.f, 0.f};
    const char* abase = smem + r16 * VPIX + q4 * 16;
#pragma unroll
    for (int ks = 0; ks < VKS; ++ks) {
      u32x4 fa[VTM];
#pragma unroll
      for (int i = 0; i < VTM; ++i) fa[i] = *reinterpret_cast<const u32x4*>(abase + i * 16 * VPIX + ks * 64);
#pragma unroll
      for (int i = 0; i < VTM; ++i)
#pragma unroll
        for (int j = 0; j < VNT; ++j) acc[i][j] = vmfma(wf[j][ks], fa[i], acc[i][j]);
    }
    if constexpr (MODE == 0) {
#pragma unroll
      for (int i = 0; i < VTM; ++i) {
        const int m = m0 + 16 * i + r16;
        long t = a.target[m < a.n ? m : a.n - 1];
        t = t < 0 ? 0 : (t >= a.V ? a.V - 1 : t);
        float x[4 * VNT], mx = -INFINITY;
#pragma unroll
        for (int j = 0; j < VNT; ++j)
#pragma unroll
          for (int e = 0; e < 4; ++e) {
            x[4 * j + e] = vok[j][e] ? acc[i][j][e] + bz[j][e] : -INFINITY;
            mx = fmaxf(mx, x[4 * j + e]);
            if (vok[j][e] && m < a.n && (long)(n0 + wid * 32 + 16 * j + 4 * q4 + e) == t) a.tgt_logit[m] = x[4 * j + e];
          }
        mx = fmaxf(mx, __shfl_xor(mx, 16, 64)); mx = fmaxf(mx, __shfl_xor(mx, 32, 64));
        float s = 0.f;
#pragma unroll
        for (int c = 0; c < 4 * VNT; ++c) s += x[c] == -INFINITY ? 0.f : __expf(x[c] - mx);
        s += __shfl_xor(s, 16, 64); s += __shfl_xor(s, 32, 64);
        if (q4 == 0) { xch[(wid * VBM + 16 * i + r16) * 2] = mx; xch[(wid * VBM + 16 * i + r16) * 2 + 1] = s; }
      }
      __syncthreads();
      if (tid < VBM && m0 + tid < a.n) {
        float M = -INFINITY, S = 0.f;
#pragma unroll
        for (int w = 0; w < 4; ++w) {
          const float mw = xch[(w * VBM + tid) * 2], sw = xch[(w * VBM + tid) * 2 + 1];
          const float nm = fmaxf(M, mw);
          S = (M == -INFINITY ? 0.f : S * __expf(M - nm)) + (mw == -INFINITY ? 0.f : sw * __expf(mw - nm));
          M = nm;
        }
        float* p = a.partial + ((size_t)nt * a.n + m0 + tid) * 2;
        p[0] = M; p[1] = S;
      }
    } else {
#pragma unroll
      for (int i = 0; i < VTM; ++i) {
        const int m = m0 + 16 * i + r16;
        const int mc = m < a.n ? m : a.n - 1;
        long t = a.target[mc];
        t = t < 0 ? 0 : (t >= a.V ? a.V - 1 : t);
        const float l = a.lse[mc];
#pragma unroll
        for (int j = 0; j < VNT; ++j) {
          float d[4];
#pragma unroll
          for (int e = 0; e < 4; ++e) {
            const int v = n0 + wid * 32 + 16 * j + 4 * q4 + e;
            const float p = vok[j][e] ? __expf(acc[i][j][e] + bz[j][e] - l) : 0.f;
            d[e] = vok[j][e] ? (p - ((long)v == t ? 1.f : 0.f)) * gs : 0.f;
          }
          if (i == 0 && j == 0) __syncthreads();
          *reinterpret_cast<u32x2*>(stage + (16 * i + r16) * VSROW + (wid * 32 + 16 * j + 4 * q4) * 2) = u32x2{pack_bf16x2(d[0], d[1]), pack_bf16x2(d[2], d[3])};
        }
      }
      __syncthreads();
#pragma unroll
      for (int i = 0; i < VBM * 16 / 256; ++i) {
        const int c = tid + 256 * i, row = c >> 4, ch = c & 15;
        const int m = m0 + row, col = n0 + ch * 8;
        if (m < a.n && col < a.ldd)
          *reinterpret_cast<u32x4*>(a.dlogits + (size_t)m * a.ldd + col) = *reinterpret_cast<const u32x4*>(stage + row * VSROW + ch * 16);
      }
    }
    __syncthreads();
    if (more) { tile_store(); __syncthreads(); }
  }
}

__global__ __launch_bounds__(256) void vocab_ce_reduce_kernel(const float* __restrict__ partial, const float* __restrict__ tgt_logit,
                                                              float* __restrict__ lse, float* __restrict__ loss, int n, int ntile, float inv_rows) {
  __shared__ float gm[4][64], gsum[4][64];
  const int tk = threadIdx.x & 63, g = threadIdx.x >> 6;
  const int m = blockIdx.x * 64 + tk, mc = m < n ? m : n - 1;
  float M = -INFINITY, S = 0.f;
  for (int j0 = g; j0 < ntile; j0 += 32) {
    float2 pj[8];
#pragma unroll
    for (int u = 0; u < 8; ++u) { const int j = j0 + 4 * u; pj[u] = *reinterpret_cast<const float2*>(partial + ((size_t)(j < ntile ? j : ntile - 1) * n + mc) * 2); }
#pragma unroll
    for (int u = 0; u < 8; ++u) {
      if (j0 + 4 * u < ntile) {
        const float mj = pj[u].x, sj = pj[u].y;
        const float nm = fmaxf(M, mj);
        S = (M == -INFINITY ? 0.f : S * __expf(M - nm)) + (mj == -INFINITY ? 0.f : sj * __expf(mj - nm));
        M = nm;
      }
    }
  }
  gm[g][tk] = M; gsum[g][tk] = S;
  __syncthreads();
  float term = 0.f;
  if (g == 0) {
    M = -INFINITY; S = 0.f;
#pragma unroll
    for (int q = 0; q < 4; ++q) {
      const float mj = gm[q][tk], sj = gsum[q][tk];
      const float nm = fmaxf(M, mj);
      S = (M == -INFINITY ? 0.f : S * __expf(M - nm)) + (mj == -INFINITY ? 0.f : sj * __expf(mj - nm));
      M = nm;
    }
    if (m < n) {
      const float l = M + __logf(S);
      lse[m] = l;
      term = (l - tgt_logit[m]) * inv_rows;
    }
#pragma unroll
    for (int o = 32; o > 0; o >>= 1) term += __shfl_xor(term, o, 64);
    if (tk == 0 && loss) atomicAdd(loss, term);
  }
}

int vce_splits(int ntile, int mtiles) {
  int s = 512 / (ntile > 0 ? ntile : 1);
  if (s < 1) s = 1;
  if (s > mtiles) s = mtiles;
  return s;
}

int vce_launch_attr() {
  static int attr_set[64] = {};
  int dev = 0;
  (void)hipGetDevice(&dev);
  if (dev >= 0 && dev < 64 && !attr_set[dev]) {
    (void)hipFuncSetAttribute(reinterpret_cast<const void*>(&vocab_ce_kernel<0>), hipFuncAttributeMaxDynamicSharedMemorySize, VLDS);
    (void)hipFuncSetAttribute(reinterpret_cast<const void*>(&vocab_ce_kernel<1>), hipFuncAttributeMaxDynamicSharedMemorySize, VLDS);
    attr_set[dev] = 1;
  }
  return 0;
}

}

int vocab_ce_supported(int dtype, int H) { return dtype == ST_BF16 && H == VH ? 1 : 0; }
int vocab_ce_tiles(int V) { return (V + VBN - 1) / VBN; }

int vocab_ce_forward(const void* y, const void* w, const float* bias, const long* target, int n, int V, float* partial, float* tgt,
                     float* lse, float* loss, hipStream_t st) {
  if (n <= 0) return 0;
  vce_launch_attr();
  VceArgs a{};
  a.y = reinterpret_cast<const bf16_t*>(y); a.w = reinterpret_cast<const bf16_t*>(w); a.bias = bias; a.target = target;
  a.partial = partial; a.tgt_logit = tgt; a.n = n; a.V = V; a.ntile = vocab_ce_tiles(V);
  a.nsplit = vce_splits(a.ntile, (n + VBM - 1) / VBM);
  hipLaunchKernelGGL(vocab_ce_kernel<0>, dim3(a.ntile * a.nsplit), dim3(256), VLDS, st, a);
  hipLaunchKernelGGL(vocab_ce_reduce_kernel, dim3((n + 63) / 64), dim3(256), 0, st, partial, tgt, lse, loss, n, a.ntile, 1.0f / n);
  ST_LAUNCH_CHECK();
  return 0;
}

int vocab_ce_dlogits(const void* y, const void* w, const float* bias, const long* target, const float* lse, int n, int V,
                     void* dlogits, int ldd, float gscale, const float* gscale_dev, hipStream_t st) {
  if (n <= 0) return 0;
  ST_CHECK(ldd % 8 == 0 && ldd >= V, "vocab_ce_dlogits: ldd=%d must be a multiple of 8 and >= V", ldd);
  vce_launch_attr();
  VceArgs a{};
  a.y = reinterpret_cast<const bf16_t*>(y); a.w = reinterpret_cast<const bf16_t*>(w); a.bias = bias; a.target = target;
  a.lse = lse; a.dlogits = reinterpret_cast<bf16_t*>(dlogits); a.gscale = gscale / n; a.gscale_dev = gscale_dev;
  a.n = n; a.V = V; a.ldd = ldd; a.ntile = (ldd + VBN - 1) / VBN;
  a.nsplit = vce_splits(a.ntile, (n + VBM - 1) / VBM);
  hipLaunchKernelGGL(vocab_ce_kernel<1>, dim3(a.ntile * a.nsplit), dim3(256), VLDS, st, a);
  ST_LAUNCH_CHECK();
  return 0;
}
```

show-tell_amd/rnn.py:

```python
import ctypes as C
import os

import torch
import torch.nn as nn

from . import _lib, ops
from ._lib import ST_BF16, ST_CELL_GRU, ST_CELL_LSTM, ST_F32, RnnGrads, RnnParams, check, lib
from .seq import plan_for

CAP_MAX = 25


def _cp(t):
    return None if t is None else C.c_void_p(t.data_ptr())


def _stream():
    return C.c_void_p(torch.cuda.current_stream().cuda_stream)


def working_copy(p, dtype):
    if dtype == torch.float32:
        return p.data
    sh = getattr(p, "_st_shadow", None)
    if (sh is None or sh.device != p.device or getattr(p, "_st_shadow_ver", -1) != p._version
            or getattr(p, "_st_shadow_ptr", 0) != p.data_ptr()):
        if sh is None or sh.device != p.device or sh.shape != p.shape:
            sh = torch.empty(p.shape, device=p.device, dtype=dtype)
        ops.cast(p.data.contiguous(), dtype, out=sh)
        p._st_shadow, p._st_shadow_ver, p._st_shadow_ptr = sh, p._version, p.data_ptr()
    return sh


def grad_buffer(p):
    if p.grad is None:
        p.grad = torch.zeros_like(p.data, dtype=torch.float32)
    return p.grad


def up8(v):
    return (v + 7) // 8 * 8


def check_sample_args(vocab_size, batch, num_samples, temperature, top_k, max_length, uniforms):
    if not temperature > 0:
        raise ValueError(f"temperature must be > 0 (got {temperature})")
    if int(top_k) != top_k or not 0 <= top_k <= min(32, vocab_size):
        raise ValueError(f"top_k must be 0 (the whole vocabulary) or 1..{min(32, vocab_size)} (got {top_k})")
    if int(num_samples) != num_samples or num_samples < 1:
        raise ValueError(f"num_samples must be >= 1 (got {num_samples})")
    if int(max_length) != max_length or max_length < 1:
        raise ValueError(f"max_length must be >= 1 (got {max_length})")
    if uniforms is not None:
        want = (batch, int(num_samples), int(max_length))
        if not torch.is_tensor(uniforms) or tuple(uniforms.shape) != want or uniforms.dtype != torch.float32:
            raise ValueError(f"uniforms must be a float32 tensor of shape {want} (images, samples, steps)")


def sample_uniforms(uniforms, shape, device, generator):
    if uniforms is not None:
        return uniforms.detach().to(device).contiguous()
    if generator is not None and generator.device.type != device.type:
        return torch.rand(shape, generator=generator, dtype=torch.float32).to(device)
    return torch.rand(shape, device=device, generator=generator, dtype=torch.float32)


def sample_lengths(ids, end_id):
    before = ((ids == end_id).cumsum(-1) == 0).sum(-1)
    return (before + 1).clamp(max=ids.shape[-1])


class _DecoderFn(torch.autograd.Function):

    @staticmethod
    def forward(ctx, feat, _anchor, module, caption, lens, mode, need_grad):
        m = module
        dev = feat.device
        if not feat.is_cuda or not m.linear.weight.is_cuda:
            raise _lib.ShowTellHipError("the decoder and its inputs must live on a HIP device (no CPU fallback in the MI355X build)")
        plan = plan_for(lens, dev)
        caption = caption.contiguous()
        seq = plan.c_struct(caption)
        prm, keep = m._c_params()
        dt = m.compute_dtype
        featd = feat.detach().contiguous()
        featd = featd if featd.dtype == dt else ops.cast(featd.float(), dt)
        nbytes = lib().st_rnn_workspace_bytes(C.byref(prm), C.byref(seq))
        ws = torch.empty(nbytes, device=dev, dtype=torch.uint8)
        V, Vp, n = m.vocab_size, lib().st_rnn_vocab_ld(m.vocab_size), plan.ntok
        targets = torch.empty(n, device=dev, dtype=torch.long)
        fused = mode == "loss" and os.environ.get("ST_FUSED_CE", "1") != "0" and bool(lib().st_rnn_fused_loss_supported(C.byref(prm)))
        logits = None if fused else torch.empty(n, Vp, device=dev, dtype=torch.float32 if mode == "logits" else dt)
        check(lib().st_rnn_forward(C.byref(prm), C.byref(seq), None, _cp(featd), _cp(ws), nbytes, _cp(logits),
                                   ST_F32 if (logits is not None and logits.dtype == torch.float32) else ST_BF16, Vp, _cp(targets),
                                   int(need_grad), _stream()), "st_rnn_forward")
        ctx.m, ctx.plan, ctx.caption, ctx.ws, ctx.mode, ctx.keep = m, plan, caption, ws, mode, keep
        ctx.feat_dtype = feat.dtype
        ctx.fused = fused
        if mode == "logits":
            return logits[:, :V]
        loss = torch.zeros((), device=dev, dtype=torch.float32)
        if fused:
            sb = lib().st_rnn_fused_loss_bytes(C.byref(prm), C.byref(seq))
            scratch = torch.empty(sb // 4, device=dev, dtype=torch.float32)
            check(lib().st_rnn_fused_loss(C.byref(prm), C.byref(seq), _cp(ws), nbytes, _cp(targets), _cp(scratch), sb, _cp(loss), _stream()),
                  "st_rnn_fused_loss")
            ctx.logits, ctx.targets, ctx.scratch = None, targets, scratch
            return loss
        check(lib().st_cross_entropy(_cp(logits), ST_F32 if dt == torch.float32 else ST_BF16, _cp(targets), n, V, Vp,
                                     _cp(loss), None, 0, Vp, 1.0, None, _stream()), "st_cross_entropy")
        ctx.logits, ctx.targets = logits, targets
        return loss

    @staticmethod
    def backward(ctx, gout):
        m, plan = ctx.m, ctx.plan
        dev = gout.device
        dt = m.compute_dtype
        dtc = ST_F32 if dt == torch.float32 else ST_BF16
        V, Vp, n = m.vocab_size, lib().st_rnn_vocab_ld(m.vocab_size), plan.ntok
        if ctx.mode == "logits":
            g = gout if gout.dtype == torch.float32 else gout.float()
            dlog = torch.zeros(n, Vp, device=dev, dtype=dt)
            gs = g.stride(0) if g.stride(1) == 1 else None
            if gs is None:
                g = g.contiguous(); gs = g.stride(0)
            check(lib().st_cast2d(_cp(g), _cp(dlog), ST_F32, dtc, n, V, gs, Vp, _stream()), "st_cast2d")
        elif ctx.fused:
            gsc = gout.detach().float().contiguous()
            dlog = torch.empty(n, Vp, device=dev, dtype=dt)
            prm_, keep_ = m._c_params()
            seq_ = plan.c_struct(ctx.caption)
            check(lib().st_rnn_fused_dlogits(C.byref(prm_), C.byref(seq_), _cp(ctx.ws), ctx.ws.numel(), _cp(ctx.targets), _cp(ctx.scratch),
                                             _cp(gsc), _cp(dlog), Vp, _stream()), "st_rnn_fused_dlogits")
        else:
            dlog = ctx.logits
            gsc = gout.detach().float().contiguous()
            check(lib().st_cross_entropy(_cp(ctx.logits), dtc, _cp(ctx.targets), n, V, Vp, None, _cp(dlog), dtc, Vp, 1.0,
                                         _cp(gsc), _stream()), "st_cross_entropy(bwd)")
        prm, keep = m._c_params()
        grads, keep2 = m._c_grads()
        seq = plan.c_struct(ctx.caption)
        dfeat = torch.empty(plan.B, m.embed_dim, device=dev, dtype=torch.float32)
        check(lib().st_rnn_backward(C.byref(prm), C.byref(grads), C.byref(seq), None, _cp(dlog), Vp, None, _cp(ctx.ws),
                                    ctx.ws.numel(), _cp(dfeat), None, _stream()), "st_rnn_backward")
        ctx.ws = None
        return dfeat.to(ctx.feat_dtype), None, None, None, None, None, None


class RNN(torch.nn.Module):

    cell = "gru"

    def __init__(self, embed_dim, num_hidden_units, vocab_size, num_layers, dtype=torch.float32):
        super(RNN, self).__init__()
        if num_layers > _lib.ST_MAX_LAYERS:
            raise ValueError(f"num_layers={num_layers} exceeds the kernel limit of {_lib.ST_MAX_LAYERS}")
        self.embeddings = nn.Embedding(vocab_size, embed_dim)
        unit_cls = nn.GRU if self.cell == "gru" else nn.LSTM
        self.unit = unit_cls(embed_dim, num_hidden_units, num_layers, batch_first=True)
        self.linear = nn.Linear(num_hidden_units, vocab_size)
        self.embed_dim, self.hidden, self.vocab_size, self.num_layers = embed_dim, num_hidden_units, vocab_size, num_layers
        self.compute_dtype = dtype

    def _layer_params(self):
        return [(getattr(self.unit, f"weight_ih_l{l}"), getattr(self.unit, f"weight_hh_l{l}"),
                 getattr(self.unit, f"bias_ih_l{l}"), getattr(self.unit, f"bias_hh_l{l}")) for l in range(self.num_layers)]

    def _c_params(self):
        dt = self.compute_dtype
        if not self.linear.weight.is_cuda:
            raise _lib.ShowTellHipError("the decoder must live on a HIP device (no CPU fallback in the MI355X build)")
        p = RnnParams()
        p.cell = ST_CELL_GRU if self.cell == "gru" else ST_CELL_LSTM
        p.dtype = ST_F32 if dt == torch.float32 else ST_BF16
        p.L, p.in0, p.H, p.V, p.E = self.num_layers, self.embed_dim, self.hidden, self.vocab_size, self.embed_dim
        keep = []
        e = working_copy(self.embeddings.weight, dt); keep.append(e); p.emb = e.data_ptr()
        for l, (wi, wh, bi, bh) in enumerate(self._layer_params()):
            a, b = working_copy(wi, dt), working_copy(wh, dt)
            keep += [a, b]
            p.w_ih[l], p.w_hh[l], p.b_ih[l], p.b_hh[l] = a.data_ptr(), b.data_ptr(), bi.data.data_ptr(), bh.data.data_ptr()
        w = working_copy(self.linear.weight, dt); keep.append(w)
        p.w_lin, p.b_lin = w.data_ptr(), self.linear.bias.data.data_ptr()
        return p, keep

    def _c_grads(self):
        g = RnnGrads()
        keep = []
        def gb(prm):
            t = grad_buffer(prm); keep.append(t); return t.data_ptr()
        g.emb = gb(self.embeddings.weight)
        for l, (wi, wh, bi, bh) in enumerate(self._layer_params()):
            g.w_ih[l], g.w_hh[l], g.b_ih[l], g.b_hh[l] = gb(wi), gb(wh), gb(bi), gb(bh)
        g.w_lin, g.b_lin = gb(self.linear.weight), gb(self.linear.bias)
        return g, keep

    def forward(self, cnn_feature, image_caption, caption_size):
        return _DecoderFn.apply(cnn_feature, self.linear.bias, self, image_caption, caption_size, "logits", torch.is_grad_enabled())

    def loss(self, cnn_feature, image_caption, caption_size):
        return _DecoderFn.apply(cnn_feature, self.linear.bias, self, image_caption, caption_size, "loss", torch.is_grad_enabled())

    def beam_search(self, cnn_feature, beam_width=4, num_hypotheses=1, max_length=50, start_id=1, end_id=2):
        from .beam import beam_search
        return beam_search(self, cnn_feature, beam_width, num_hypotheses, max_length, start_id, end_id)

    def sample(self, cnn_feature, num_samples=1, temperature=1.0, top_k=0, max_length=CAP_MAX, end_id=2, generator=None,
               uniforms=None):
        B, S, T = cnn_feature.shape[0], num_samples, max_length
        check_sample_args(self.vocab_size, B, S, temperature, top_k, T, uniforms)
        S, T = int(S), int(T)
        with torch.no_grad():
            prm, keep = self._c_params()
            if not cnn_feature.is_cuda:
                raise _lib.ShowTellHipError("cnn_feature must be on the HIP device (no CPU fallback)")
            dt = self.compute_dtype
            feat = cnn_feature.detach().contiguous()
            feat = feat if feat.dtype == dt else ops.cast(feat.float(), dt)
            if S > 1:
                feat = feat.repeat_interleave(S, 0)
            n, dev = B * S, feat.device
            u = sample_uniforms(uniforms, (B, S, T), dev, generator)
            nbytes = lib().st_rnn_sample_workspace_bytes(C.byref(prm), n)
            ws = torch.empty(nbytes, device=dev, dtype=torch.uint8)
            ids = torch.empty(n, T, device=dev, dtype=torch.long)
            logp = torch.empty(n, T, device=dev, dtype=torch.float32)
            check(lib().st_rnn_sample(C.byref(prm), _cp(feat), n, T, _cp(u), 1.0 / float(temperature), int(top_k), int(end_id), _cp(ws),
                                      nbytes, _cp(ids), _cp(logp), _stream()), "st_rnn_sample")
            return ids.view(B, S, T), logp.view(B, S, T), sample_lengths(ids, end_id).view(B, S)

    def sentence_index(self, cnn_feature, beam_size=0, return_logits=False):
        if beam_size and beam_size > 0:
            from .beam import quirky_beam
            return quirky_beam(self, cnn_feature, beam_size)
        with torch.no_grad():
            prm, keep = self._c_params()
            dt = self.compute_dtype
            feat = cnn_feature.detach().contiguous()
            feat = feat if feat.dtype == dt else ops.cast(feat.float(), dt)
            B = feat.shape[0]
            nbytes = lib().st_rnn_greedy_workspace_bytes(C.byref(prm), B)
            ws = torch.empty(nbytes, device=feat.device, dtype=torch.uint8)
            ids = torch.empty(B, CAP_MAX, device=feat.device, dtype=torch.long)
            lg = torch.empty(CAP_MAX, B, up8(self.vocab_size), device=feat.device) if return_logits else None
            check(lib().st_rnn_greedy(C.byref(prm), _cp(feat), B, CAP_MAX, _cp(ws), nbytes, _cp(ids), _cp(lg), _stream()),
                  "st_rnn_greedy")
        out = ids.squeeze()
        if return_logits:
            return out, lg[:, :, :self.vocab_size].permute(1, 0, 2)
        return out
```

Baseline: 32080 images/sec.

## Fuse vocab projection weight gradient into fused dlogits kernel; coalesce forward GRU loads

Adds a vocab CE backward kernel that computes the dlogits tile and, in the same pass, accumulates the linear-layer weight and bias gradients with MFMA, writing them out with atomics. This removes the separate transpose, colsum and NT GEMM from the RNN backward. Separately, the teacher-forced forward GRU GEMM now uses the coalesced weight-load lane mapping, and two workspace memsets are merged into one. The atomics make results nondeterministic, and the merged memset assumes the two workspace regions are contiguous.

```diff
diff --git a/include/showtell_hip.h b/include/showtell_hip.h
--- a/include/showtell_hip.h
+++ b/include/showtell_hip.h
@@ -231,6 +231,9 @@
                       const long* targets, float* scratch, size_t scratch_bytes, float* loss_accum, void* stream);
 int st_rnn_fused_dlogits(const st_rnn_params* p, const st_packed_seq* s, const void* workspace, size_t workspace_bytes,
                          const long* targets, const float* scratch, const float* grad_scale_dev, void* dlogits, int ldd, void* stream);
+int st_rnn_fused_dlogits_dw(const st_rnn_params* p, const st_packed_seq* s, const void* workspace, size_t workspace_bytes,
+                            const long* targets, const float* scratch, const float* grad_scale_dev, void* dlogits, int ldd,
+                            float* dw_lin, float* db_lin, void* stream);
 
 int st_cross_entropy(const void* logits, int logits_dtype, const long* target, int rows, int V, int ldl,
                      float* loss_accum, void* dlogits, int dlogits_dtype, int ldd, float grad_scale,
diff --git a/show-tell_amd/_lib.py b/show-tell_amd/_lib.py
--- a/show-tell_amd/_lib.py
+++ b/show-tell_amd/_lib.py
@@ -157,6 +157,7 @@
     "st_rnn_fused_loss_bytes": ([C.POINTER(RnnParams), C.POINTER(PackedSeq)], C.c_size_t),
     "st_rnn_fused_loss": ([C.POINTER(RnnParams), C.POINTER(PackedSeq), c_p, C.c_size_t, c_p, c_p, C.c_size_t, c_p, c_p], c_i),
     "st_rnn_fused_dlogits": ([C.POINTER(RnnParams), C.POINTER(PackedSeq), c_p, C.c_size_t, c_p, c_p, c_p, c_p, c_i, c_p], c_i),
+    "st_rnn_fused_dlogits_dw": ([C.POINTER(RnnParams), C.POINTER(PackedSeq), c_p, C.c_size_t, c_p, c_p, c_p, c_p, c_i, c_p, c_p, c_p], c_i),
     "st_rnn_backward": ([C.POINTER(RnnParams), C.POINTER(RnnGrads), C.POINTER(PackedSeq), c_p, c_p, c_i, c_p, c_p, C.c_size_t,
                          c_p, c_p, c_p], c_i),
     "st_rnn_greedy_workspace_bytes": ([C.POINTER(RnnParams), c_i], C.c_size_t),
diff --git a/show-tell_amd/csrc/rnn.cpp b/show-tell_amd/csrc/rnn.cpp
--- a/show-tell_amd/csrc/rnn.cpp
+++ b/show-tell_amd/csrc/rnn.cpp
@@ -100,7 +100,7 @@
                                   t > 0 ? cl + (size_t)off[t - 1] * H * es : nullptr, yl + (size_t)off[t] * H * es, cl + (size_t)off[t] * H * es,
                                   bt, save_for_backward ? gl + (size_t)off[t] * 4 * H * es : nullptr);
     }
-    if (rnn_gemm_launch_batch(cells, nc, dt, rnn_cell_epi(p->cell), 1, st)) return 1;
+    if (rnn_gemm_launch_batch(cells, nc, dt, rnn_cell_epi(p->cell), 1, st, 1)) return 1;
   }
   if (logits) {
     ST_CHECK(p->w_lin && p->b_lin, "st_rnn_forward: logits requested without the vocabulary projection");
@@ -139,6 +139,19 @@
   const char* ytop = reinterpret_cast<const char*>(workspace) + q.y + (size_t)(p->L - 1) * s->ntok * p->H * q.es;
   return vocab_ce_dlogits(ytop, p->w_lin, p->b_lin, targets, scratch, s->ntok, p->V, dlogits, ldd, 1.0f, grad_scale_dev,
                           reinterpret_cast<hipStream_t>(stream));
+}
+
+extern "C" int st_rnn_fused_dlogits_dw(const st_rnn_params* p, const st_packed_seq* s, const void* workspace, size_t workspace_bytes,
+                                       const long* targets, const float* scratch, const float* grad_scale_dev, void* dlogits, int ldd,
+                                       float* dw_lin, float* db_lin, void* stream) {
+  if (check_common(p, s, "st_rnn_fused_dlogits_dw")) return 1;
+  ST_CHECK(workspace && targets && scratch && dlogits && dw_lin && db_lin, "st_rnn_fused_dlogits_dw: null pointer");
+  ST_CHECK(st_rnn_fused_loss_supported(p), "st_rnn_fused_dlogits_dw: unsupported configuration");
+  const Plan q = make_plan(p, s);
+  ST_CHECK(workspace_bytes >= q.total, "st_rnn_fused_dlogits_dw: workspace too small");
+  const char* ytop = reinterpret_cast<const char*>(workspace) + q.y + (size_t)(p->L - 1) * s->ntok * p->H * q.es;
+  return vocab_ce_dlogits_dw(ytop, p->w_lin, p->b_lin, targets, scratch, s->ntok, p->V, dlogits, ldd, 1.0f, grad_scale_dev, dw_lin, db_lin,
+                             reinterpret_cast<hipStream_t>(stream));
 }
 
 extern "C" int st_rnn_backward(const st_rnn_params* p, const st_rnn_grads* g, const st_packed_seq* s,
@@ -159,12 +172,15 @@
   const char* ytop = ws + q.y + (size_t)(p->L - 1) * n * H * es;
 
   if (dlogits) {
-    ST_CHECK(p->w_lin && g->w_lin && g->b_lin, "st_rnn_backward: vocabulary projection gradients requested without buffers");
+    const bool lin_done = !g->w_lin && !g->b_lin;
+    ST_CHECK(p->w_lin && (lin_done || (g->w_lin && g->b_lin)), "st_rnn_backward: vocabulary projection gradients requested without buffers");
     ST_CHECK(ldd >= st_up8(p->V) && ldd % 8 == 0 && ldd <= q.Vp, "st_rnn_backward: dlogits leading dimension %d must be a multiple of 8 in [%d, %d]",
              ldd, st_up8(p->V), q.Vp);
-    if (st_transpose_colsum(dlogits, ws + q.tA, g->b_lin, dt, n, p->V, ldd, Np, stream)) return 1;
-    if (st_transpose(ytop, ws + q.tB, dt, n, H, H, Np, stream)) return 1;
-    if (st_gemm_nt(ws + q.tA, Np, ws + q.tB, Np, g->w_lin, H, p->V, H, Np, dt, ST_F32, nullptr, stream, 1)) return 1;
+    if (!lin_done) {
+      if (st_transpose_colsum(dlogits, ws + q.tA, g->b_lin, dt, n, p->V, ldd, Np, stream)) return 1;
+      if (st_transpose(ytop, ws + q.tB, dt, n, H, H, Np, stream)) return 1;
+      if (st_gemm_nt(ws + q.tA, Np, ws + q.tB, Np, g->w_lin, H, p->V, H, Np, dt, ST_F32, nullptr, stream, 1)) return 1;
+    }
     if (st_transpose(p->w_lin, ws + q.wT, dt, p->V, H, H, ldd, stream)) return 1;
     const int bk = dt == ST_BF16 ? 64 : 32;
     const int split = (ldd % (8 * bk) == 0 && ldd >= 16 * bk) ? 8 : 0;
@@ -187,8 +203,7 @@
   auto dccl = [&](int l) { return reinterpret_cast<float*>(ws + q.dcc) + (size_t)l * s->B * H; };
   auto wThh = [&](int l) { return ws + q.wThh + (size_t)l * H * GH * es; };
   auto wTih = [&](int l) { return ws + q.wTih + (size_t)l * q.maxw * GH * es; };
-  if (hipMemsetAsync(ws + q.dhc, 0, (size_t)L * s->B * H * sizeof(float), st) != hipSuccess ||
-      hipMemsetAsync(ws + q.dcc, 0, (size_t)L * s->B * H * sizeof(float), st) != hipSuccess) { st_set_error("memset failed"); return 1; }
+  if (hipMemsetAsync(ws + q.dhc, 0, q.dcc - q.dhc + (size_t)L * s->B * H * sizeof(float), st) != hipSuccess) { st_set_error("memset failed"); return 1; }
   {
     const void* wx[2][ST_MAX_LAYERS]; void* wy[2][ST_MAX_LAYERS];
     int ni = 0;
diff --git a/show-tell_amd/csrc/rnn_kernels.h b/show-tell_amd/csrc/rnn_kernels.h
--- a/show-tell_amd/csrc/rnn_kernels.h
+++ b/show-tell_amd/csrc/rnn_kernels.h
@@ -54,9 +54,11 @@
                      float* lse, float* loss, hipStream_t st);
 int vocab_ce_dlogits(const void* y, const void* w, const float* bias, const long* target, const float* lse, int n, int V,
                      void* dlogits, int ldd, float gscale, const float* gscale_dev, hipStream_t st);
+int vocab_ce_dlogits_dw(const void* y, const void* w, const float* bias, const long* target, const float* lse, int n, int V,
+                        void* dlogits, int ldd, float gscale, const float* gscale_dev, float* dw, float* db, hipStream_t st);
 
 int rnn_gemm_launch(const RnnGemmArgs& a, int dtype, int epi, int has_x, hipStream_t st);
-int rnn_gemm_launch_batch(const RnnGemmArgs* cells, int ncells, int dtype, int epi, int has_x, hipStream_t st);
+int rnn_gemm_launch_batch(const RnnGemmArgs* cells, int ncells, int dtype, int epi, int has_x, hipStream_t st, int teacher_forced = 0);
 int rnn_bwd_gates_launch_batch(const RnnBwdCell* cells, int ncells, int H, int cell_kind, int dtype, hipStream_t st);
 int rnn_bwd_fused_launch_batch(const RnnBwdFused* cells, int ncells, int cell_kind, int dtype, hipStream_t st);
 int pack_inputs_launch(const void* feat, const void* emb, const long* cap, int Tcap, const int* rows_b, const int* rows_t,
diff --git a/show-tell_amd/csrc/rnn_kernels.hip b/show-tell_amd/csrc/rnn_kernels.hip
--- a/show-tell_amd/csrc/rnn_kernels.hip
+++ b/show-tell_amd/csrc/rnn_kernels.hip
@@ -1,5 +1,6 @@
 #include "common.h"
 #include "rnn_kernels.h"
+#include <stdlib.h>
 #include <string.h>
 
 namespace {
@@ -45,12 +46,12 @@
   return u32x4{(unsigned)__builtin_amdgcn_ds_bpermute(src4, (int)v[0]), (unsigned)__builtin_amdgcn_ds_bpermute(src4, (int)v[1]),
                (unsigned)__builtin_amdgcn_ds_bpermute(src4, (int)v[2]), (unsigned)__builtin_amdgcn_ds_bpermute(src4, (int)v[3])};
 }
-template <typename T, int NG, bool HAS_X, int MT, bool BWD = false>
+template <typename T, int NG, bool HAS_X, int MT, bool BWD = false, bool COAL = BWD>
 __device__ __forceinline__ void skinny_mma(const RnnGemmArgs& a, int mbase, int n0, int r16, int q4, int kslice,
                                            f32x4 (&accH)[MT][NG], f32x4 (&accX)[MT][NG]) {
   constexpr int EPC = Mfma<T>::EPC;
   constexpr int UNR = BWD ? (MT + NG <= 4 ? 4 : 2) : (HAS_X && MT == 2) ? 2 : 4;
-  const int lr = BWD ? q4 * 4 + (r16 >> 2) : r16, lq = BWD ? (r16 & 3) : q4;
+  const int lr = COAL ? q4 * 4 + (r16 >> 2) : r16, lq = COAL ? (r16 & 3) : q4;
   const int n = n0 + lr;
   const bool nok = n < a.N;
   const bool hasH = a.A != nullptr, hasX = HAS_X && a.A2 != nullptr;
@@ -70,7 +71,7 @@
       if (mok[t]) {
         tok = (int)(0xffffffffu - (unsigned)(a.x_keys[m] & 0xffffffffull));
         if (tok < 0 || tok >= a.x_V) tok = 0;
-        if (a.ids_out && n0 == 0 && kslice == 0 && q4 == 0) a.ids_out[(long)m * a.ids_stride + a.ids_t] = tok;
+        if (a.ids_out && n0 == 0 && kslice == 0 && lq == 0) a.ids_out[(long)m * a.ids_stride + a.ids_t] = tok;
       }
       AH[t] = reinterpret_cast<const T*>(a.A) + (long)tok * a.lda;
     }
@@ -80,7 +81,7 @@
       if (mok[t]) {
         tok = (int)(0xffffffffu - (unsigned)(a.x_keys[m] & 0xffffffffull));
         if (tok < 0 || tok >= a.x_V) tok = 0;
-        if (a.ids_out && n0 == 0 && kslice == 0 && q4 == 0) a.ids_out[(long)m * a.ids_stride + a.ids_t] = tok;
+        if (a.ids_out && n0 == 0 && kslice == 0 && lq == 0) a.ids_out[(long)m * a.ids_stride + a.ids_t] = tok;
       }
       xrow = tok;
     }
@@ -121,7 +122,7 @@
         }
       }
     }
-    if (BWD) {
+    if (COAL) {
       const int src4 = (r16 * 4 + q4) * 4;
 #pragma unroll
       for (int u = 0; u < UNR; ++u) {
@@ -143,7 +144,7 @@
   }
 }
 
-template <typename T, int NG, int EPI, bool HAS_X, int MT>
+template <typename T, int NG, int EPI, bool HAS_X, int MT, bool COAL = false>
 __global__ __launch_bounds__(256) void rnn_gemm_kernel(RnnGemmBatch batch) {
   const RnnGemmArgs& a = batch.c[blockIdx.z];
   __shared__ f32x4 red[4][MT][2 * NG][64];
@@ -181,7 +182,7 @@
       if (prev && a.accumulate != kCellRawOut) load4<T>(reinterpret_cast<const T*>(prev) + (long)pm * a.ldhp + pn, es);
     }
   }
-  skinny_mma<T, NG, HAS_X, MT>(a, mbase, n0, r16, q4, wid, accH, accX);
+  skinny_mma<T, NG, HAS_X, MT, false, COAL>(a, mbase, n0, r16, q4, wid, accH, accX);
 #pragma unroll
   for (int t = 0; t < MT; ++t)
 #pragma unroll
@@ -580,15 +581,17 @@
 
 }
 
-int rnn_gemm_launch_batch(const RnnGemmArgs* cells, int ncells, int dtype, int epi, int has_x, hipStream_t st) {
+int rnn_gemm_launch_batch(const RnnGemmArgs* cells, int ncells, int dtype, int epi, int has_x, hipStream_t st, int teacher_forced) {
   ST_CHECK(ncells >= 0 && ncells <= kRnnBatch, "rnn_gemm: %d cells in one launch (max %d)", ncells, kRnnBatch);
   RnnGemmBatch b;
   memset(&b, 0, sizeof(b));
   const int epc = dtype == ST_BF16 ? 8 : 4;
   int nc = 0, maxM = 0, maxN = 0;
+  bool keyed = false;
   for (int i = 0; i < ncells; ++i) {
     const RnnGemmArgs& a = cells[i];
     if (a.M <= 0) continue;
+    if (a.x_keys) keyed = true;
     ST_CHECK(epi == 3 || a.N % 4 == 0, "rnn_gemm: N=%d must be a multiple of 4", a.N);
     ST_CHECK(a.K % epc == 0 && a.lda % epc == 0 && a.ldw % epc == 0, "rnn_gemm: K/lda/ldw must be multiples of %d", epc);
     if (has_x) ST_CHECK(a.K2 % epc == 0 && a.lda2 % epc == 0 && a.ldw2 % epc == 0, "rnn_gemm: K2/lda2/ldw2 must be multiples of %d", epc);
@@ -600,19 +603,23 @@
   const dim3 grid((maxN + 15) / 16, (maxM + 15) / 16, nc), block(256);
   const bool mt2 = (nc >= 2 || maxM >= 512) && maxM > 16 && epi != 3;
   const dim3 grid2((maxN + 15) / 16, (maxM + 31) / 32, nc);
-#define RG(T, NG, EPI, HX) do { if (mt2) hipLaunchKernelGGL((rnn_gemm_kernel<T, NG, EPI, HX, 2>), grid2, block, 0, st, b); \
-                               else hipLaunchKernelGGL((rnn_gemm_kernel<T, NG, EPI, HX, 1>), grid, block, 0, st, b); } while (0)
+  const char* env = getenv("ST_FWD_COALESCE");
+  const bool coal = teacher_forced && has_x && (epi == 1 || epi == 2) && !keyed && !(env && env[0] == '0');
+#define RG(T, NG, EPI, HX, CO) do { if (mt2) hipLaunchKernelGGL((rnn_gemm_kernel<T, NG, EPI, HX, 2, CO>), grid2, block, 0, st, b); \
+                                   else hipLaunchKernelGGL((rnn_gemm_kernel<T, NG, EPI, HX, 1, CO>), grid, block, 0, st, b); } while (0)
+#define RGX(T, NG, EPI) do { if (!has_x) RG(T, NG, EPI, false, false); else if (coal) RG(T, NG, EPI, true, true); else RG(T, NG, EPI, true, false); } while (0)
   if (dtype == ST_BF16) {
-    if (epi == 0) RG(bf16_t, 1, 0, false);
-    else if (epi == 3) RG(bf16_t, 1, 3, false);
-    else if (epi == 1) { if (has_x) RG(bf16_t, 3, 1, true); else RG(bf16_t, 3, 1, false); }
-    else { if (has_x) RG(bf16_t, 4, 2, true); else RG(bf16_t, 4, 2, false); }
+    if (epi == 0) RG(bf16_t, 1, 0, false, false);
+    else if (epi == 3) RG(bf16_t, 1, 3, false, false);
+    else if (epi == 1) RGX(bf16_t, 3, 1);
+    else RGX(bf16_t, 4, 2);
   } else {
-    if (epi == 0) RG(float, 1, 0, false);
-    else if (epi == 3) RG(float, 1, 3, false);
-    else if (epi == 1) { if (has_x) RG(float, 3, 1, true); else RG(float, 3, 1, false); }
-    else { if (has_x) RG(float, 4, 2, true); else RG(float, 4, 2, false); }
-  }
+    if (epi == 0) RG(float, 1, 0, false, false);
+    else if (epi == 3) RG(float, 1, 3, false, false);
+    else if (epi == 1) RGX(float, 3, 1);
+    else RGX(float, 4, 2);
+  }
+#undef RGX
 #undef RG
   ST_LAUNCH_CHECK();
   return 0;
diff --git a/show-tell_amd/csrc/vocab_ce.hip b/show-tell_amd/csrc/vocab_ce.hip
--- a/show-tell_amd/csrc/vocab_ce.hip
+++ b/show-tell_amd/csrc/vocab_ce.hip
@@ -213,6 +213,139 @@
   }
 }
 
+constexpr int WBN = 64;
+constexpr int WSROW = WBN * 2 + 16;
+constexpr int WLDS = 2 * VTILE + VBM * WSROW;
+
+typedef short s16x4 __attribute__((ext_vector_type(4)));
+__device__ __forceinline__ u32x2 lds_read_tr16(const char* p) {
+  const s16x4 v = __builtin_amdgcn_ds_read_tr16_b64_v4i16((__attribute__((address_space(3))) s16x4*)p);
+  return *reinterpret_cast<const u32x2*>(&v);
+}
+
+struct VceDwArgs { VceArgs a; float* dw; float* db; };
+
+__global__ __launch_bounds__(256, 2) void vocab_ce_dw_kernel(VceDwArgs g) {
+  const VceArgs& a = g.a;
+  extern __shared__ __attribute__((aligned(16))) char smem[];
+  char* stage = smem + 2 * VTILE;
+  const int tid = threadIdx.x, lane = tid & 63;
+  const int wid = __builtin_amdgcn_readfirstlane(tid >> 6);
+  const int r16 = lane & 15, q4 = lane >> 4;
+  const int mtiles = (a.n + VBM - 1) / VBM;
+  const int nt = blockIdx.x / a.nsplit, sp = blockIdx.x - nt * a.nsplit;
+  const int n0 = nt * WBN;
+  if (sp >= mtiles) return;
+
+  auto row_request = [&](int mt, int i) {
+    int m = mt * VBM + (tid >> 6) + 4 * i; m = m < a.n ? m : a.n - 1;
+    return *reinterpret_cast<const u32x4*>(a.y + (size_t)m * VH + (tid & 63) * 8);
+  };
+  auto row_store = [&](char* tile, int i, const u32x4& v) { *reinterpret_cast<u32x4*>(tile + ((tid >> 6) + 4 * i) * VPIX + (tid & 63) * 16) = v; };
+  {
+    u32x4 tv[VNL];
+#pragma unroll
+    for (int i = 0; i < VNL; ++i) tv[i] = row_request(sp, i);
+#pragma unroll
+    for (int i = 0; i < VNL; ++i) row_store(smem, i, tv[i]);
+  }
+  u32x4 wf[VKS];
+  {
+    int r = n0 + wid * 16 + r16; r = r < a.V ? r : a.V - 1;
+    const bf16_t* wp = a.w + (size_t)r * VH + q4 * 8;
+#pragma unroll
+    for (int ks = 0; ks < VKS; ++ks) wf[ks] = *reinterpret_cast<const u32x4*>(wp + ks * 32);
+  }
+  float bz[4]; bool vok[4];
+#pragma unroll
+  for (int e = 0; e < 4; ++e) {
+    const int v = n0 + wid * 16 + 4 * q4 + e;
+    vok[e] = v < a.V;
+    bz[e] = vok[e] ? a.bias[v] : 0.f;
+  }
+  float gs = a.gscale;
+  if (a.gscale_dev) gs *= *a.gscale_dev;
+  f32x4 dw[VH / 16];
+#pragma unroll
+  for (int ht = 0; ht < VH / 16; ++ht) dw[ht] = f32x4{0.f, 0.f, 0.f, 0.f};
+  float dbs[4] = {0.f, 0.f, 0.f, 0.f};
+  const int trow = 4 * q4 + (r16 >> 2), tcol = 4 * (r16 & 3);
+  const char* sA = stage + trow * WSROW + (wid * 16 + tcol) * 2;
+  __syncthreads();
+
+  int it = 0;
+  for (int mt = sp; mt < mtiles; mt += a.nsplit, ++it) {
+    const int m0 = mt * VBM;
+    const bool more = mt + a.nsplit < mtiles;
+    const char* cur = smem + (it & 1) * VTILE;
+    char* nxt = smem + ((it & 1) ^ 1) * VTILE;
+    f32x4 acc[VTM];
+#pragma unroll
+    for (int i = 0; i < VTM; ++i) acc[i] = f32x4{0.f, 0.f, 0.f, 0.f};
+    const char* abase = cur + r16 * VPIX + q4 * 16;
+#pragma unroll
+    for (int ks = 0; ks < VKS; ++ks) {
+      u32x4 fa[VTM];
+#pragma unroll
+      for (int i = 0; i < VTM; ++i) fa[i] = *reinterpret_cast<const u32x4*>(abase + i * 16 * VPIX + ks * 64);
+#pragma unroll
+      for (int i = 0; i < VTM; ++i) acc[i] = vmfma(wf[ks], fa[i], acc[i]);
+    }
+#pragma unroll
+    for (int i = 0; i < VTM; ++i) {
+      const int m = m0 + 16 * i + r16;
+      const int mc = m < a.n ? m : a.n - 1;
+      long t = a.target[mc];
+      t = t < 0 ? 0 : (t >= a.V ? a.V - 1 : t);
+      const float l = a.lse[mc];
+      float d[4];
+#pragma unroll
+      for (int e = 0; e < 4; ++e) {
+        const int v = n0 + wid * 16 + 4 * q4 + e;
+        const float p = vok[e] ? __expf(acc[i][e] + bz[e] - l) : 0.f;
+        d[e] = vok[e] && m < a.n ? (p - ((long)v == t ? 1.f : 0.f)) * gs : 0.f;
+      }
+      const u32x2 pk = u32x2{pack_bf16x2(d[0], d[1]), pack_bf16x2(d[2], d[3])};
+      dbs[0] += __uint_as_float(pk[0] << 16); dbs[1] += __uint_as_float(pk[0] & 0xffff0000u);
+      dbs[2] += __uint_as_float(pk[1] << 16); dbs[3] += __uint_as_float(pk[1] & 0xffff0000u);
+      *reinterpret_cast<u32x2*>(stage + (16 * i + r16) * WSROW + (wid * 16 + 4 * q4) * 2) = pk;
+    }
+    __syncthreads();
+    {
+      const int row = tid >> 3, ch = tid & 7;
+      const int m = m0 + row, col = n0 + ch * 8;
+      if (m < a.n && col < a.ldd)
+        *reinterpret_cast<u32x4*>(a.dlogits + (size_t)m * a.ldd + col) = *reinterpret_cast<const u32x4*>(stage + row * WSROW + ch * 16);
+    }
+    const u32x2 a0 = lds_read_tr16(sA), a1 = lds_read_tr16(sA + 16 * WSROW);
+    const u32x4 fd = u32x4{a0[0], a0[1], a1[0], a1[1]};
+    const char* sB = cur + trow * VPIX + tcol * 2;
+    u32x4 tv[2];
+#pragma unroll
+    for (int ht = 0; ht < VH / 16; ++ht) {
+      const int i0 = (ht >> 3) * 2;
+      if ((ht & 7) == 0 && more) { tv[0] = row_request(mt + a.nsplit, i0); tv[1] = row_request(mt + a.nsplit, i0 + 1); }
+      const u32x2 b0 = lds_read_tr16(sB + ht * 32), b1 = lds_read_tr16(sB + 16 * VPIX + ht * 32);
+      dw[ht] = vmfma(fd, u32x4{b0[0], b0[1], b1[0], b1[1]}, dw[ht]);
+      if ((ht & 7) == 7 && more) { row_store(nxt, i0, tv[0]); row_store(nxt, i0 + 1, tv[1]); }
+    }
+    __syncthreads();
+  }
+#pragma unroll
+  for (int e = 0; e < 4; ++e) {
+    const int v = n0 + wid * 16 + 4 * q4 + e;
+    float s = dbs[e];
+#pragma unroll
+    for (int o = 1; o < 16; o <<= 1) s += __shfl_xor(s, o, 64);
+    if (v < a.V) {
+      float* row = g.dw + (size_t)v * VH + r16;
+#pragma unroll
+      for (int ht = 0; ht < VH / 16; ++ht) unsafeAtomicAdd(row + ht * 16, dw[ht][e]);
+      if (r16 == 0) unsafeAtomicAdd(g.db + v, s);
+    }
+  }
+}
+
 int vce_splits(int ntile, int mtiles) {
   int s = 512 / (ntile > 0 ? ntile : 1);
   if (s < 1) s = 1;
@@ -227,6 +360,7 @@
   if (dev >= 0 && dev < 64 && !attr_set[dev]) {
     (void)hipFuncSetAttribute(reinterpret_cast<const void*>(&vocab_ce_kernel<0>), hipFuncAttributeMaxDynamicSharedMemorySize, VLDS);
     (void)hipFuncSetAttribute(reinterpret_cast<const void*>(&vocab_ce_kernel<1>), hipFuncAttributeMaxDynamicSharedMemorySize, VLDS);
+    (void)hipFuncSetAttribute(reinterpret_cast<const void*>(&vocab_ce_dw_kernel), hipFuncAttributeMaxDynamicSharedMemorySize, WLDS);
     attr_set[dev] = 1;
   }
   return 0;
@@ -265,3 +399,20 @@
   ST_LAUNCH_CHECK();
   return 0;
 }
+
+int vocab_ce_dlogits_dw(const void* y, const void* w, const float* bias, const long* target, const float* lse, int n, int V,
+                        void* dlogits, int ldd, float gscale, const float* gscale_dev, float* dw, float* db, hipStream_t st) {
+  if (n <= 0) return 0;
+  ST_CHECK(ldd % 8 == 0 && ldd >= V, "vocab_ce_dlogits_dw: ldd=%d must be a multiple of 8 and >= V", ldd);
+  vce_launch_attr();
+  VceDwArgs g{};
+  VceArgs& a = g.a;
+  a.y = reinterpret_cast<const bf16_t*>(y); a.w = reinterpret_cast<const bf16_t*>(w); a.bias = bias; a.target = target;
+  a.lse = lse; a.dlogits = reinterpret_cast<bf16_t*>(dlogits); a.gscale = gscale / n; a.gscale_dev = gscale_dev;
+  a.n = n; a.V = V; a.ldd = ldd; a.ntile = (ldd + WBN - 1) / WBN;
+  a.nsplit = (n + VBM - 1) / VBM >= 2 ? 2 : 1;
+  g.dw = dw; g.db = db;
+  hipLaunchKernelGGL(vocab_ce_dw_kernel, dim3(a.ntile * a.nsplit), dim3(256), WLDS, st, g);
+  ST_LAUNCH_CHECK();
+  return 0;
+}
diff --git a/show-tell_amd/rnn.py b/show-tell_amd/rnn.py
--- a/show-tell_amd/rnn.py
+++ b/show-tell_amd/rnn.py
@@ -119,6 +119,7 @@
         dt = m.compute_dtype
         dtc = ST_F32 if dt == torch.float32 else ST_BF16
         V, Vp, n = m.vocab_size, lib().st_rnn_vocab_ld(m.vocab_size), plan.ntok
+        lin_fused = False
         if ctx.mode == "logits":
             g = gout if gout.dtype == torch.float32 else gout.float()
             dlog = torch.zeros(n, Vp, device=dev, dtype=dt)
@@ -131,8 +132,15 @@
             dlog = torch.empty(n, Vp, device=dev, dtype=dt)
             prm_, keep_ = m._c_params()
             seq_ = plan.c_struct(ctx.caption)
-            check(lib().st_rnn_fused_dlogits(C.byref(prm_), C.byref(seq_), _cp(ctx.ws), ctx.ws.numel(), _cp(ctx.targets), _cp(ctx.scratch),
-                                             _cp(gsc), _cp(dlog), Vp, _stream()), "st_rnn_fused_dlogits")
+            lin_fused = os.environ.get("ST_VOCAB_BWD_FUSED", "1") != "0"
+            if lin_fused:
+                gw, gb = grad_buffer(m.linear.weight), grad_buffer(m.linear.bias)
+                check(lib().st_rnn_fused_dlogits_dw(C.byref(prm_), C.byref(seq_), _cp(ctx.ws), ctx.ws.numel(), _cp(ctx.targets),
+                                                    _cp(ctx.scratch), _cp(gsc), _cp(dlog), Vp, _cp(gw), _cp(gb), _stream()),
+                      "st_rnn_fused_dlogits_dw")
+            else:
+                check(lib().st_rnn_fused_dlogits(C.byref(prm_), C.byref(seq_), _cp(ctx.ws), ctx.ws.numel(), _cp(ctx.targets),
+                                                 _cp(ctx.scratch), _cp(gsc), _cp(dlog), Vp, _stream()), "st_rnn_fused_dlogits")
         else:
             dlog = ctx.logits
             gsc = gout.detach().float().contiguous()
@@ -140,6 +148,8 @@
                                          _cp(gsc), _stream()), "st_cross_entropy(bwd)")
         prm, keep = m._c_params()
         grads, keep2 = m._c_grads()
+        if lin_fused:
+            grads.w_lin = grads.b_lin = None
         seq = plan.c_struct(ctx.caption)
         dfeat = torch.empty(plan.B, m.embed_dim, device=dev, dtype=torch.float32)
         check(lib().st_rnn_backward(C.byref(prm), C.byref(grads), C.byref(seq), None, _cp(dlog), Vp, None, _cp(ctx.ws),
```

After: 32320 images/sec, median of 6. No clear change (+0.7%).
